# lucidrains/vit-pytorch

Hardware: AMD Instinct MI355X
Metric: images/sec (fwd+bwd) ViT-B/16 224^2 bf16 (higher is better)
Workload: dtype bf16

## Files before the change

include/vitk.h:

```cpp
#ifndef VITK_H
#define VITK_H

#include <stdint.h>
#include <stddef.h>

#ifdef __cplusplus
extern "C" {
#endif

#define VITK_VERSION 138

#define VITK_F32 0
#define VITK_BF16 1
#define VITK_F16 2

#define VITK_E_ARG (-1)
#define VITK_E_SHAPE (-2)
#define VITK_E_ALIGN (-3)
#define VITK_E_DTYPE (-4)
#define VITK_E_UNAVAILABLE (-5)
#define VITK_E_COMM (-6)

int vitk_version(void);
int vitk_half_type(void);
const char* vitk_last_error(void);

typedef struct vitk_rowmap { int64_t group, gstride, offset; } vitk_rowmap;

int vitk_layernorm_fwd(const void* x, int xdt, const void* w, const void* b, int wdt,
                       void* y, int ydt, float* mean, float* rstd,
                       int64_t rows, int64_t D, float eps,
                       vitk_rowmap imap, vitk_rowmap omap,
                       const void* add, int64_t add_group, int64_t add_off, void* stream);

int64_t vitk_layernorm_bwd_blocks(int64_t rows, int64_t D);
int vitk_layernorm_bwd(const void* dy, int dydt, const void* x, int xdt, const void* w, int wdt,
                       const float* mean, const float* rstd,
                       const float* gin, float* dx_f32, void* dx_t, int dxtdt,
                       float* partials, int colsum_dx,
                       int64_t rows, int64_t D,
                       vitk_rowmap dymap, vitk_rowmap xmap, vitk_rowmap dxmap, void* stream);
int vitk_layernorm_bwd_drop(const void* dy, int dydt, const void* x, int xdt, const void* w, int wdt,
                            const float* mean, const float* rstd, const float* gin, float* dx_f32, void* dx_t, int dxtdt,
                            float* partials, int colsum_dx, int64_t rows, int64_t D, vitk_rowmap dymap, vitk_rowmap xmap,
                            vitk_rowmap dxmap, float drop_p, uint32_t drop_seed, void* stream);
int vitk_layernorm_bwd_s16(const void* dy, int dydt, const void* x, int xdt, const void* w, int wdt, const float* mean,
                           const float* rstd, const void* gin, void* dx_t, int dxtdt, float* partials, int colsum_dx,
                           int64_t rows, int64_t D, vitk_rowmap dymap, vitk_rowmap xmap, vitk_rowmap dxmap, void* stream);

int vitk_layernorm_bwd_finalize(const float* partials, int64_t nblk, int64_t D, void* dw, void* db, int odt,
                                float* dcol, void* stream);
int vitk_layernorm_bwd_finalize_ex(const float* partials, int64_t nblk, int64_t D, void* dw, void* db, int odt,
                                   void* dcol, int dcol_dt, void* stream);

int vitk_colsum_partials(const float* partials, int64_t nparts, int64_t ld, int64_t cols,
                         void* out, int odt, int accumulate, void* stream);

int64_t vitk_colsum_ws_floats(int64_t rows, int64_t cols);
int vitk_colsum(const void* x, int xdt, int64_t rows, int64_t cols, int64_t ld,
                void* out, int odt, int accumulate, float* ws, void* stream);

#define VITK_EPI_NONE 0
#define VITK_EPI_BIAS 1
#define VITK_EPI_BIAS_GELU 2
#define VITK_EPI_RESID 3
#define VITK_EPI_RESID16 5
#define VITK_EPI_GELU_BWD 4
#define VITK_EPI_BIAS_GELU_DG 6
#define VITK_EPI_MUL_AUX 7
#define VITK_EPI_BIAS_GELU_DG8 8
#define VITK_EPI_MUL_AUX8 9

int vitk_gemm_nt_bf16(const void* A, int64_t lda, const void* W, int64_t ldw,
                      void* C, int64_t ldc, int64_t M, int64_t N, int64_t K,
                      int epilogue, const void* bias, const float* resid, void* aux, void* stream);

int64_t vitk_gemm_nt_colsum_rows(int64_t M, int64_t N, int64_t K, int64_t ldc);
int vitk_gemm_nt_bf16_mul_aux_colsum(const void* A, int64_t lda, const void* W, int64_t ldw, void* C, int64_t ldc,
                                     int64_t M, int64_t N, int64_t K, const void* aux, float* colsum_partials, void* stream);
int vitk_gemm_nt_bf16_mul_aux8_colsum(const void* A, int64_t lda, const void* W, int64_t ldw, void* C, int64_t ldc,
                                      int64_t M, int64_t N, int64_t K, const void* aux8, float* colsum_partials, void* stream);
int vitk_gemm_nt_plan(int64_t M, int64_t N, int64_t K, int64_t ldc, int32_t* out5);
int64_t vitk_pack_w_nt_bytes(int64_t rows, int64_t reduction);
int vitk_pack_w_nt(const void* W, int64_t ldw, int64_t N, int64_t K, void* out, void* out_t, void* stream);
int vitk_pack_w_nt_many(const void* const* W, const int64_t* ldw, const int64_t* N, const int64_t* K, void* const* out,
                        void* const* out_t, int64_t count, void* stream);
int vitk_gemm_nt_bf16_gelu_bwd_colsum(const void* A, int64_t lda, const void* W, int64_t ldw,
                                      void* C, int64_t ldc, int64_t M, int64_t N, int64_t K,
                                      void* aux, float* colsum_partials, void* stream);
int vitk_gemm_nt_bf16_drop(const void* A, int64_t lda, const void* W, int64_t ldw, void* C, int64_t ldc, int64_t M, int64_t N,
                           int64_t K, int epilogue, const void* bias, const float* resid, void* aux, float* colsum_partials,
                           float drop_p, uint32_t drop_seed, void* stream);

int vitk_gemm_nt_fp8(const void* A8, int64_t lda, const void* W8, int64_t ldw, void* C, int64_t ldc, int64_t M, int64_t N,
                     int64_t K, int epilogue, const void* bias, const float* resid, void* aux, float alpha, void* stream);
int vitk_fp8_amax_scale(const void* x, int dt, int64_t n, float* scale2, void* stream);
int vitk_quantize_fp8(const void* x, int dt, void* out, int64_t n, const float* scale_dev, float scale_host, void* stream);
int vitk_layernorm_fwd_fp8(const void* x, int xdt, const void* w, const void* b, int wdt, void* y, int ydt,
                           float* mean, float* rstd, int64_t rows, int64_t D, float eps, vitk_rowmap imap, vitk_rowmap omap,
                           const void* add, int64_t add_group, int64_t add_off, void* y8, const float* scale8,
                           uint32_t* amax64, void* stream);
int vitk_gemm_nt_fp8_ex(const void* A, int64_t lda, int a_is_fp8, const void* W, int64_t ldw, void* C, int64_t ldc, int64_t M,
                        int64_t N, int64_t K, int epilogue, const void* bias, const float* resid, void* aux, float alpha,
                        const float* alpha_a, const float* alpha_w, void* c8, const float* c8_scale, uint32_t* c8_amax64,
                        void* stream);
int vitk_fp8_update_scales(uint32_t* amax64, float* scales2, int64_t nslots, void* stream);
int vitk_gemm_nt_fp8_v2(const void* A, int64_t lda, int a_kind, const void* W, int64_t ldw, void* C, int64_t ldc, int64_t M,
                        int64_t N, int64_t K, int epilogue, const void* bias, const float* resid, void* aux,
                        float* colsum_partials, float alpha, const float* alpha_a, const float* alpha_w, void* c8,
                        const float* c8_scale, uint32_t* c8_amax64, int flags, void* stream);
int64_t vitk_gemm_nt_fp8_colsum_rows(int64_t M, int64_t N, int64_t K, int64_t ldc);
int vitk_quantize_fp8_delayed(const void* x, int dt, void* out8, int64_t n, const float* scale2, uint32_t* amax64, int fmt,
                              void* stream);
int vitk_fp8_update_scales_fmt(uint32_t* amax64, float* scales2, int64_t nslots, const float* fmax, void* stream);
int64_t vitk_gemm_tn_fp8_splits(int64_t M, int64_t N, int64_t K, int flags);
int vitk_gemm_tn_fp8(const void* dY8, int64_t ldy, const void* X8, int64_t ldx, void* dW, int odt, int64_t ldo, int accumulate,
                     int64_t M, int64_t N, int64_t K, float* ws, int64_t splits, const float* alpha_y, const float* alpha_x,
                     int flags, void* stream);

int64_t vitk_gemm_tn_splits(int64_t M, int64_t N, int64_t K);
int vitk_set_cu_reserve(int cus);
int vitk_get_cu_reserve(void);
int vitk_test_occupy_cus(int ncus, float ms, void* stream);
int vitk_gemm_tn_bf16(const void* dY, int64_t ldy, const void* X, int64_t ldx,
                      void* dW, int odt, int64_t ldo, int accumulate,
                      int64_t M, int64_t N, int64_t K, float* ws, int64_t splits, void* stream);
int64_t vitk_gemm_tn_pair_splits(int64_t M, int64_t N0, int64_t K0, int64_t N1, int64_t K1);
int vitk_gemm_tn_bf16_pair(const void* dY0, int64_t ldy0, const void* X0, int64_t ldx0, void* dW0, int64_t ldo0, int accumulate0,
                           int64_t N0, int64_t K0, const void* dY1, int64_t ldy1, const void* X1, int64_t ldx1, void* dW1,
                           int64_t ldo1, int accumulate1, int64_t N1, int64_t K1, int odt, int64_t M, float* ws, int64_t splits,
                           void* stream);

typedef struct vitk_mat { const void* p; int dt; int64_t s_b1, s_b2, s_row, s_col; } vitk_mat;
int vitk_gemm_generic(vitk_mat A, vitk_mat B, vitk_mat C, const void* bias, int bias_dt,
                      int64_t nb1, int64_t nb2, int64_t M, int64_t N, int64_t K,
                      float alpha, float beta, void* stream);

typedef struct vitk_bhnd { void* p; int64_t s_b, s_h, s_n; } vitk_bhnd;
int vitk_attn_fwd_bf16(vitk_bhnd q, vitk_bhnd k, vitk_bhnd v, vitk_bhnd o, float* lse,
                       int64_t B, int64_t H, int64_t N, int64_t d, float scale, void* stream);
int vitk_attn_bwd_bf16(vitk_bhnd q, vitk_bhnd k, vitk_bhnd v, vitk_bhnd o, vitk_bhnd dout,
                       const float* lse, float* delta,
                       vitk_bhnd dq, vitk_bhnd dk, vitk_bhnd dv,
                       int64_t B, int64_t H, int64_t N, int64_t d, float scale, void* stream);
int vitk_attn_fwd_bf16_drop(vitk_bhnd q, vitk_bhnd k, vitk_bhnd v, vitk_bhnd o, float* lse, int64_t B, int64_t H,
                            int64_t N, int64_t d, float scale, float drop_p, uint32_t drop_seed, void* stream);
int vitk_attn_bwd_bf16_drop(vitk_bhnd q, vitk_bhnd k, vitk_bhnd v, vitk_bhnd o, vitk_bhnd dout, const float* lse,
                            float* delta, vitk_bhnd dq, vitk_bhnd dk, vitk_bhnd dv, int64_t B, int64_t H, int64_t N,
                            int64_t d, float scale, float drop_p, uint32_t drop_seed, void* stream);
int vitk_split2(const float* x, void* hi, void* lo, int64_t n, void* stream);
int vitk_attn_fwd_x2(vitk_bhnd q_hi, vitk_bhnd q_lo, vitk_bhnd k_hi, vitk_bhnd k_lo, vitk_bhnd v_hi, vitk_bhnd v_lo, vitk_bhnd o_f32,
                     float* lse, int64_t B, int64_t H, int64_t N, int64_t d, float scale, void* stream);
int vitk_attn_bwd_x2(vitk_bhnd q_hi, vitk_bhnd q_lo, vitk_bhnd k_hi, vitk_bhnd k_lo, vitk_bhnd v_hi, vitk_bhnd v_lo, vitk_bhnd o_f32,
                     vitk_bhnd do_hi, vitk_bhnd do_lo, const float* lse, float* delta, vitk_bhnd dq_f32, vitk_bhnd dk_f32,
                     vitk_bhnd dv_f32, int64_t B, int64_t H, int64_t N, int64_t d, float scale, void* stream);
int vitk_dropout_keep(uint8_t* keep, int64_t rows, int64_t cols, float p, uint32_t seed, void* stream);

typedef struct vitk_hnd { void* p; int64_t s_h, s_n; } vitk_hnd;
int vitk_attn_varlen_fwd_bf16(vitk_hnd q, vitk_hnd k, vitk_hnd v, vitk_hnd o, float* lse,
                              const int32_t* cu_q, const int32_t* cu_k, const int32_t* blk_seg, const int32_t* blk_r0,
                              int64_t nblk, int64_t tq_total, int64_t H, int64_t d, float scale, void* stream);
int vitk_attn_varlen_bwd_bf16(vitk_hnd q, vitk_hnd k, vitk_hnd v, vitk_hnd o, vitk_hnd dout, const float* lse, float* delta,
                              vitk_hnd dq, vitk_hnd dk, vitk_hnd dv, const int32_t* cu_q, const int32_t* cu_k,
                              const int32_t* qblk_seg, const int32_t* qblk_r0, int64_t nqblk,
                              const int32_t* kblk_seg, const int32_t* kblk_r0, int64_t nkblk,
                              int64_t tq_total, int64_t H, int64_t d, float scale, void* stream);
int vitk_attn_varlen_fwd_bf16_drop(vitk_hnd q, vitk_hnd k, vitk_hnd v, vitk_hnd o, float* lse,
                                   const int32_t* cu_q, const int32_t* cu_k, const int32_t* blk_seg, const int32_t* blk_r0,
                                   int64_t nblk, int64_t tq_total, int64_t H, int64_t d, float scale, float drop_p,
                                   uint32_t drop_seed, void* stream);
int vitk_attn_varlen_bwd_bf16_drop(vitk_hnd q, vitk_hnd k, vitk_hnd v, vitk_hnd o, vitk_hnd dout, const float* lse, float* delta,
                                   vitk_hnd dq, vitk_hnd dk, vitk_hnd dv, const int32_t* cu_q, const int32_t* cu_k,
                                   const int32_t* qblk_seg, const int32_t* qblk_r0, int64_t nqblk,
                                   const int32_t* kblk_seg, const int32_t* kblk_r0, int64_t nkblk,
                                   int64_t tq_total, int64_t H, int64_t d, float scale, float drop_p, uint32_t drop_seed,
                                   void* stream);

int64_t vitk_rmsnorm_heads_rows(int64_t T, int64_t H);
int vitk_rmsnorm_heads_fwd(const void* x, int64_t ldx, const void* gamma, void* y, int64_t ldy, float* rnorm, int dt,
                           int64_t T, int64_t H, int64_t d, void* stream);
int vitk_rmsnorm_heads_bwd(const void* dy, int64_t lddy, const void* x, int64_t ldx, const void* gamma, const float* rnorm,
                           void* dx, int64_t lddx, void* dgamma, float* partials, int dt,
                           int64_t T, int64_t H, int64_t d, void* stream);

int vitk_softmax_fwd(const void* s, void* p, int dt, int64_t rows, int64_t cols, float scale, void* stream);
int vitk_softmax_bwd(const void* p, const void* dp, void* ds, int dt, int64_t rows, int64_t cols,
                     float scale, void* stream);

int vitk_patchify(const void* img, void* out, int dt, int64_t B, int64_t C, int64_t H, int64_t W,
                  int64_t p1, int64_t p2, void* stream);
int vitk_unpatchify(const void* dpatch, void* dimg, int dt, int64_t B, int64_t C, int64_t H, int64_t W,
                    int64_t p1, int64_t p2, void* stream);
int vitk_patch_ln_serves(int dt, int64_t C, int64_t H, int64_t W, int64_t p1, int64_t p2);
int64_t vitk_patch_ln_bwd_blocks(int64_t rows);
int vitk_patch_ln_fwd(const void* img, int dt, const void* w, const void* b, void* y, float* mean, float* rstd, int64_t B,
                      int64_t C, int64_t H, int64_t W, int64_t p1, int64_t p2, float eps, void* stream);
int vitk_patch_ln_bwd_params(const void* dy, const void* img, int dt, const float* mean, const float* rstd, float* partials,
                             int64_t B, int64_t C, int64_t H, int64_t W, int64_t p1, int64_t p2, void* stream);
int vitk_patchify_cpp(const void* img, void* out, int dt, int64_t C, int64_t H, int64_t W, int64_t p,
                      int64_t row0, int64_t ld, void* stream);
int vitk_unpatchify_cpp(const void* dpatch, void* dimg, int dt, int64_t C, int64_t H, int64_t W, int64_t p,
                        int64_t row0, int64_t ld, void* stream);
int vitk_gather_add2(const void* x, const void* A, const int32_t* ia, const void* B, const int32_t* ib, void* out, int dt,
                     int64_t T, int64_t D, void* stream);
int vitk_csr_rowsum(const void* g, int gdt, const int32_t* ptr, const int32_t* rows, void* out, int odt,
                    int64_t nseg, int64_t D, void* stream);
int vitk_gelu_fwd(const void* x, void* y, int dt, int64_t n, void* stream);
int vitk_gelu_bwd(const void* dy, const void* x, void* dx, int dt, int64_t n, void* stream);
int vitk_add_rows(const void* a, int adt, const void* b, int bdt, const void* bias, int biasdt,
                  void* out, int odt, int64_t rows, int64_t cols, void* stream);
int vitk_cast(const void* x, int xdt, void* y, int ydt, int64_t n, void* stream);
int vitk_cast_many(const void* const* src, void* const* dst, const int64_t* numel, int64_t count, int xdt, int ydt, void* stream);
int vitk_fold_many(const float* const* src, void* const* dst, const int64_t* nparts, const int64_t* ld, const int64_t* cols,
                   const int32_t* flags, int64_t count, void* stream);
int vitk_write_cls_rows(void* x, int xdt, const void* cls, const void* pos, int pdt,
                        int64_t B, int64_t N, int64_t D, int64_t ncls, void* stream);
int vitk_mean_pool_fwd(const void* x, int xdt, void* out, int odt, int64_t B, int64_t N, int64_t D, void* stream);
int vitk_mean_pool_bwd(const void* dout, int ddt, void* dx, int xdt, int64_t B, int64_t N, int64_t D, void* stream);
int vitk_dropout_fwd(const void* x, void* y, uint8_t* mask, int dt, int64_t n, float p,
                     uint64_t seed, uint64_t offset, void* stream);
int vitk_dropout_bwd(const void* dy, const uint8_t* mask, void* dx, int dt, int64_t n, float p, void* stream);
int vitk_copy_cols(const void* src, int64_t ld_src, void* dst, int64_t ld_dst, int dt, int64_t rows, int64_t cols_copy,
                   int64_t cols_dst, void* stream);
int vitk_split_bf16x3(const float* x, int64_t ldx, void* out, int64_t ld_out, int64_t block_stride, int64_t rows,
                      int64_t cols, int operand_b, void* stream);
int vitk_concat_tokens(const void* x, const void* front, const void* pos, void* out, int dt, int64_t B, int64_t Np,
                       int64_t F, int64_t D, void* stream);
int vitk_gather_tokens(const void* src, const int32_t* idx, void* dst, int dt, int64_t B, int64_t Np, int64_t Kp, int64_t D,
                       int scatter, void* stream);
int vitk_adam_step(void* param, const void* grad, int dt, float* exp_avg, float* exp_avg_sq, float* master, int64_t n,
                   float lr, float beta1, float beta2, float eps, float weight_decay, int decoupled, int64_t step,
                   float grad_scale, void* stream);
int vitk_transpose(const void* in, void* out, int dt, int64_t rows, int64_t cols, void* stream);

#define VITK_COMM_ID_BYTES 128
typedef void* vitk_comm_t;
int vitk_comm_unique_id(void* out128);
int vitk_comm_init(const void* id128, int rank, int world, vitk_comm_t* out);
int vitk_comm_allreduce(vitk_comm_t comm, void* buf, int64_t n, int dt, int average, void* stream);
int vitk_comm_destroy(vitk_comm_t comm);

#ifdef __cplusplus
}
#endif
#endif
```

vit_pytorch_amd/_lib.py:

```python
from __future__ import annotations

import ctypes as C
import os
import threading

HERE = os.path.dirname(os.path.abspath(__file__))
LIB_PATH = os.environ.get("VITK_LIB") or os.path.join(HERE, "libvitk.so")
LIB_PATH_F16 = (os.path.join(os.path.dirname(LIB_PATH), os.path.basename(LIB_PATH).replace("libvitk", "libvitk_f16", 1)) if os.environ.get("VITK_LIB")
                else os.path.join(HERE, "libvitk_f16.so"))

F32, BF16 = 0, 1
HALF_TYPE_F16 = 2
EPI_NONE, EPI_BIAS, EPI_BIAS_GELU, EPI_RESID, EPI_GELU_BWD, EPI_RESID16, EPI_BIAS_GELU_DG, EPI_MUL_AUX = 0, 1, 2, 3, 4, 5, 6, 7
EPI_BIAS_GELU_DG8, EPI_MUL_AUX8 = 8, 9
VITK_VERSION = 138


class RowMap(C.Structure):
    _fields_ = [("group", C.c_int64), ("gstride", C.c_int64), ("offset", C.c_int64)]


class Mat(C.Structure):
    _fields_ = [("p", C.c_void_p), ("dt", C.c_int), ("s_b1", C.c_int64), ("s_b2", C.c_int64),
                ("s_row", C.c_int64), ("s_col", C.c_int64)]


class HND(C.Structure):
    _fields_ = [("p", C.c_void_p), ("s_h", C.c_int64), ("s_n", C.c_int64)]


class BHND(C.Structure):
    _fields_ = [("p", C.c_void_p), ("s_b", C.c_int64), ("s_h", C.c_int64), ("s_n", C.c_int64)]


IDENT = RowMap(0, 0, 0)

_vp, _i, _i64, _f, _u64 = C.c_void_p, C.c_int, C.c_int64, C.c_float, C.c_uint64

SIGNATURES = {
    "vitk_version": (_i, []),
    "vitk_last_error": (C.c_char_p, []),
    "vitk_layernorm_fwd": (_i, [_vp, _i, _vp, _vp, _i, _vp, _i, _vp, _vp, _i64, _i64, _f, RowMap, RowMap, _vp, _i64, _i64, _vp]),
    "vitk_layernorm_bwd_blocks": (_i64, [_i64, _i64]),
    "vitk_layernorm_bwd": (_i, [_vp, _i, _vp, _i, _vp, _i, _vp, _vp, _vp, _vp, _vp, _i, _vp, _i, _i64, _i64, RowMap, RowMap, RowMap, _vp]),
    "vitk_layernorm_bwd_finalize": (_i, [_vp, _i64, _i64, _vp, _vp, _i, _vp, _vp]),
    "vitk_layernorm_bwd_finalize_ex": (_i, [_vp, _i64, _i64, _vp, _vp, _i, _vp, _i, _vp]),
    "vitk_colsum_partials": (_i, [_vp, _i64, _i64, _i64, _vp, _i, _i, _vp]),
    "vitk_colsum_ws_floats": (_i64, [_i64, _i64]),
    "vitk_colsum": (_i, [_vp, _i, _i64, _i64, _i64, _vp, _i, _i, _vp, _vp]),
    "vitk_gemm_nt_bf16": (_i, [_vp, _i64, _vp, _i64, _vp, _i64, _i64, _i64, _i64, _i, _vp, _vp, _vp, _vp]),
    "vitk_half_type": (_i, []),
    "vitk_adam_step": (_i, [_vp, _vp, _i, _vp, _vp, _vp, _i64, _f, _f, _f, _f, _f, _i, _i64, _f, _vp]),
    "vitk_gemm_nt_bf16_drop": (_i, [_vp, _i64, _vp, _i64, _vp, _i64, _i64, _i64, _i64, _i, _vp, _vp, _vp, _vp, _f, C.c_uint32, _vp]),
    "vitk_layernorm_bwd_drop": (_i, [_vp, _i, _vp, _i, _vp, _i, _vp, _vp, _vp, _vp, _vp, _i, _vp, _i, _i64, _i64, RowMap, RowMap, RowMap, _f, C.c_uint32, _vp]),
    "vitk_layernorm_bwd_s16": (_i, [_vp, _i, _vp, _i, _vp, _i, _vp, _vp, _vp, _vp, _i, _vp, _i, _i64, _i64, RowMap, RowMap, RowMap, _vp]),
    "vitk_gemm_nt_fp8": (_i, [_vp, _i64, _vp, _i64, _vp, _i64, _i64, _i64, _i64, _i, _vp, _vp, _vp, _f, _vp]),
    "vitk_fp8_amax_scale": (_i, [_vp, _i, _i64, _vp, _vp]),
    "vitk_quantize_fp8": (_i, [_vp, _i, _vp, _i64, _vp, _f, _vp]),
    "vitk_layernorm_fwd_fp8": (_i, [_vp, _i, _vp, _vp, _i, _vp, _i, _vp, _vp, _i64, _i64, _f, RowMap, RowMap, _vp, _i64, _i64, _vp, _vp, _vp, _vp]),
    "vitk_gemm_nt_fp8_ex": (_i, [_vp, _i64, _i, _vp, _i64, _vp, _i64, _i64, _i64, _i64, _i, _vp, _vp, _vp, _f, _vp, _vp, _vp, _vp, _vp, _vp]),
    "vitk_fp8_update_scales": (_i, [_vp, _vp, _i64, _vp]),
    "vitk_gemm_nt_fp8_v2": (_i, [_vp, _i64, _i, _vp, _i64, _vp, _i64, _i64, _i64, _i64, _i, _vp, _vp, _vp, _vp, _f, _vp, _vp, _vp, _vp, _vp, _i, _vp]),
    "vitk_gemm_nt_fp8_colsum_rows": (_i64, [_i64, _i64, _i64, _i64]),
    "vitk_quantize_fp8_delayed": (_i, [_vp, _i, _vp, _i64, _vp, _vp, _i, _vp]),
    "vitk_fp8_update_scales_fmt": (_i, [_vp, _vp, _i64, _vp, _vp]),
    "vitk_gemm_tn_fp8_splits": (_i64, [_i64, _i64, _i64, _i]),
    "vitk_gemm_tn_fp8": (_i, [_vp, _i64, _vp, _i64, _vp, _i, _i64, _i, _i64, _i64, _i64, _vp, _i64, _vp, _vp, _i, _vp]),
    "vitk_gemm_nt_colsum_rows": (_i64, [_i64, _i64, _i64, _i64]),
    "vitk_gemm_nt_plan": (_i, [_i64, _i64, _i64, _i64, _vp]),
    "vitk_comm_unique_id": (_i, [_vp]),
    "vitk_comm_init": (_i, [_vp, _i, _i, _vp]),
    "vitk_comm_allreduce": (_i, [_vp, _vp, _i64, _i, _i, _vp]),
    "vitk_comm_destroy": (_i, [_vp]),
    "vitk_pack_w_nt_bytes": (_i64, [_i64, _i64]),
    "vitk_pack_w_nt": (_i, [_vp, _i64, _i64, _i64, _vp, _vp, _vp]),
    "vitk_pack_w_nt_many": (_i, [_vp, _vp, _vp, _vp, _vp, _vp, _i64, _vp]),
    "vitk_gemm_nt_bf16_gelu_bwd_colsum": (_i, [_vp, _i64, _vp, _i64, _vp, _i64, _i64, _i64, _i64, _vp, _vp, _vp]),
    "vitk_gemm_nt_bf16_mul_aux_colsum": (_i, [_vp, _i64, _vp, _i64, _vp, _i64, _i64, _i64, _i64, _vp, _vp, _vp]),
    "vitk_gemm_nt_bf16_mul_aux8_colsum": (_i, [_vp, _i64, _vp, _i64, _vp, _i64, _i64, _i64, _i64, _vp, _vp, _vp]),
    "vitk_gemm_tn_splits": (_i64, [_i64, _i64, _i64]),
    "vitk_set_cu_reserve": (_i, [_i]),
    "vitk_get_cu_reserve": (_i, []),
    "vitk_test_occupy_cus": (_i, [_i, _f, _vp]),
    "vitk_gemm_tn_bf16": (_i, [_vp, _i64, _vp, _i64, _vp, _i, _i64, _i, _i64, _i64, _i64, _vp, _i64, _vp]),
    "vitk_gemm_tn_pair_splits": (_i64, [_i64, _i64, _i64, _i64, _i64]),
    "vitk_gemm_tn_bf16_pair": (_i, [_vp, _i64, _vp, _i64, _vp, _i64, _i, _i64, _i64, _vp, _i64, _vp, _i64, _vp, _i64, _i, _i64, _i64, _i, _i64, _vp, _i64, _vp]),
    "vitk_gemm_generic": (_i, [Mat, Mat, Mat, _vp, _i, _i64, _i64, _i64, _i64, _i64, _f, _f, _vp]),
    "vitk_attn_fwd_bf16": (_i, [BHND, BHND, BHND, BHND, _vp, _i64, _i64, _i64, _i64, _f, _vp]),
    "vitk_attn_bwd_bf16": (_i, [BHND, BHND, BHND, BHND, BHND, _vp, _vp, BHND, BHND, BHND, _i64, _i64, _i64, _i64, _f, _vp]),
    "vitk_attn_fwd_bf16_drop": (_i, [BHND, BHND, BHND, BHND, _vp, _i64, _i64, _i64, _i64, _f, _f, C.c_uint32, _vp]),
    "vitk_attn_bwd_bf16_drop": (_i, [BHND, BHND, BHND, BHND, BHND, _vp, _vp, BHND, BHND, BHND, _i64, _i64, _i64, _i64, _f, _f, C.c_uint32, _vp]),
    "vitk_split2": (_i, [_vp, _vp, _vp, _i64, _vp]),
    "vitk_attn_fwd_x2": (_i, [BHND] * 7 + [_vp, _i64, _i64, _i64, _i64, _f, _vp]),
    "vitk_attn_bwd_x2": (_i, [BHND] * 9 + [_vp, _vp, BHND, BHND, BHND, _i64, _i64, _i64, _i64, _f, _vp]),
    "vitk_dropout_keep": (_i, [_vp, _i64, _i64, _f, C.c_uint32, _vp]),
    "vitk_attn_varlen_fwd_bf16": (_i, [HND, HND, HND, HND, _vp, _vp, _vp, _vp, _vp, _i64, _i64, _i64, _i64, _f, _vp]),
    "vitk_attn_varlen_bwd_bf16": (_i, [HND, HND, HND, HND, HND, _vp, _vp, HND, HND, HND, _vp, _vp, _vp, _vp, _i64, _vp, _vp, _i64, _i64, _i64, _i64, _f, _vp]),
    "vitk_attn_varlen_fwd_bf16_drop": (_i, [HND, HND, HND, HND, _vp, _vp, _vp, _vp, _vp, _i64, _i64, _i64, _i64, _f, _f, C.c_uint32, _vp]),
    "vitk_attn_varlen_bwd_bf16_drop": (_i, [HND, HND, HND, HND, HND, _vp, _vp, HND, HND, HND, _vp, _vp, _vp, _vp, _i64, _vp, _vp, _i64, _i64, _i64, _i64, _f, _f, C.c_uint32, _vp]),
    "vitk_rmsnorm_heads_rows": (_i64, [_i64, _i64]),
    "vitk_rmsnorm_heads_fwd": (_i, [_vp, _i64, _vp, _vp, _i64, _vp, _i, _i64, _i64, _i64, _vp]),
    "vitk_rmsnorm_heads_bwd": (_i, [_vp, _i64, _vp, _i64, _vp, _vp, _vp, _i64, _vp, _vp, _i, _i64, _i64, _i64, _vp]),
    "vitk_softmax_fwd": (_i, [_vp, _vp, _i, _i64, _i64, _f, _vp]),
    "vitk_softmax_bwd": (_i, [_vp, _vp, _vp, _i, _i64, _i64, _f, _vp]),
    "vitk_patchify": (_i, [_vp, _vp, _i, _i64, _i64, _i64, _i64, _i64, _i64, _vp]),
    "vitk_unpatchify": (_i, [_vp, _vp, _i, _i64, _i64, _i64, _i64, _i64, _i64, _vp]),
    "vitk_patchify_cpp": (_i, [_vp, _vp, _i, _i64, _i64, _i64, _i64, _i64, _i64, _vp]),
    "vitk_unpatchify_cpp": (_i, [_vp, _vp, _i, _i64, _i64, _i64, _i64, _i64, _i64, _vp]),
    "vitk_patch_ln_serves": (_i, [_i, _i64, _i64, _i64, _i64, _i64]),
    "vitk_patch_ln_bwd_blocks": (_i64, [_i64]),
    "vitk_patch_ln_fwd": (_i, [_vp, _i, _vp, _vp, _vp, _vp, _vp, _i64, _i64, _i64, _i64, _i64, _i64, _f, _vp]),
    "vitk_patch_ln_bwd_params": (_i, [_vp, _vp, _i, _vp, _vp, _vp, _i64, _i64, _i64, _i64, _i64, _i64, _vp]),
    "vitk_gather_add2": (_i, [_vp, _vp, _vp, _vp, _vp, _vp, _i, _i64, _i64, _vp]),
    "vitk_csr_rowsum": (_i, [_vp, _i, _vp, _vp, _vp, _i, _i64, _i64, _vp]),
    "vitk_gelu_fwd": (_i, [_vp, _vp, _i, _i64, _vp]),
    "vitk_gelu_bwd": (_i, [_vp, _vp, _vp, _i, _i64, _vp]),
    "vitk_add_rows": (_i, [_vp, _i, _vp, _i, _vp, _i, _vp, _i, _i64, _i64, _vp]),
    "vitk_cast": (_i, [_vp, _i, _vp, _i, _i64, _vp]),
    "vitk_cast_many": (_i, [_vp, _vp, _vp, _i64, _i, _i, _vp]),
    "vitk_fold_many": (_i, [_vp, _vp, _vp, _vp, _vp, _vp, _i64, _vp]),
    "vitk_write_cls_rows": (_i, [_vp, _i, _vp, _vp, _i, _i64, _i64, _i64, _i64, _vp]),
    "vitk_mean_pool_fwd": (_i, [_vp, _i, _vp, _i, _i64, _i64, _i64, _vp]),
    "vitk_mean_pool_bwd": (_i, [_vp, _i, _vp, _i, _i64, _i64, _i64, _vp]),
    "vitk_dropout_fwd": (_i, [_vp, _vp, _vp, _i, _i64, _f, _u64, _u64, _vp]),
    "vitk_dropout_bwd": (_i, [_vp, _vp, _vp, _i, _i64, _f, _vp]),
    "vitk_copy_cols": (_i, [_vp, _i64, _vp, _i64, _i, _i64, _i64, _i64, _vp]),
    "vitk_split_bf16x3": (_i, [_vp, _i64, _vp, _i64, _i64, _i64, _i64, _i, _vp]),
    "vitk_concat_tokens": (_i, [_vp, _vp, _vp, _vp, _i, _i64, _i64, _i64, _i64, _vp]),
    "vitk_gather_tokens": (_i, [_vp, _vp, _vp, _i, _i64, _i64, _i64, _i64, _i, _vp]),
    "vitk_transpose": (_i, [_vp, _vp, _i, _i64, _i64, _vp]),
}

_lib = None
_lib_f16 = None


class VitkError(RuntimeError):
    pass


def _open(path: str, half_type: int):
    if not os.path.exists(path):
        raise VitkError(
            f"{path} not found: the HIP kernel library is not built. "
            "Build it with `python -c 'import __graft_entry__ as g; g.build()'` "
            "(or `python -m vit_pytorch_amd._build`). There is no CPU/eager fallback.")
    import torch
    lib = C.CDLL(path)
    for name, (res, args) in SIGNATURES.items():
        fn = getattr(lib, name)
        fn.restype = res
        fn.argtypes = args
    v = lib.vitk_version()
    if v != VITK_VERSION:
        raise VitkError(f"{os.path.basename(path)} version {v} != binding version {VITK_VERSION}; rebuild")
    if lib.vitk_half_type() != half_type:
        raise VitkError(f"{os.path.basename(path)} was built for the wrong 16-bit type; rebuild")
    return lib


def load():
    global _lib
    if _lib is None:
        _lib = _open(LIB_PATH, BF16)
    return _lib


def load_f16():
    global _lib_f16
    if _lib_f16 is None:
        _lib_f16 = _open(LIB_PATH_F16, HALF_TYPE_F16)
    return _lib_f16


_tls = threading.local()


def note_last_lib(lib):
    _tls.lib = lib


def check(rc: int, what: str = ""):
    if rc != 0:
        msg = (getattr(_tls, "lib", None) or load()).vitk_last_error().decode("utf-8", "replace")
        raise VitkError(f"{what}: vitk error {rc}: {msg}")
```

vit_pytorch_amd/csrc/gemm_bf16.hip:

```cpp
#include "common.h"
#include <atomic>
#include "gemm_nt_plan.h"
#include <stdlib.h>

namespace {

constexpr int BM = 128, BN = 128;
constexpr int NT_BK = 32;
constexpr int NT_TILE_BYTES = 128 * NT_BK * 2;
constexpr int NT_STAGE_BYTES = 2 * NT_TILE_BYTES;
constexpr int NXCD = 8;

__device__ __forceinline__ int xcd_swizzle(int b, int nwg) {
    const int q = nwg / NXCD, r = nwg % NXCD;
    const int xcd = b % NXCD, idx = b / NXCD;
    return (xcd < r ? xcd * (q + 1) : r * (q + 1) + (xcd - r) * q) + idx;
}

__device__ __forceinline__ void grouped_tile(int wg, int tiles_m, int tiles_n, int gn, int& tm, int& tn) {
    const int per_group = gn * tiles_m;
    const int g = wg / per_group;
    const int r = wg - g * per_group;
    const int rem = tiles_n - g * gn;
    const int w = rem < gn ? rem : gn;
    tm = r / w;
    tn = g * gn + (r - tm * w);
}

__device__ __forceinline__ int swz_f(int x) { return (0x1320 >> (4 * (x & 3))) & 3; }

template <int EPI>
__global__ __launch_bounds__(256) void gemm_nt_kernel(
    const __bf16* __restrict__ A, long long lda, const __bf16* __restrict__ W, long long ldw,
    void* __restrict__ Cv, long long ldc, int M, int N, int K,
    const __bf16* __restrict__ bias, const float* __restrict__ resid, __bf16* __restrict__ aux,
    int tiles_n, int nwg) {
    __shared__ __attribute__((aligned(16))) char lds[2 * NT_STAGE_BYTES];

    const int tid = threadIdx.x;
    const int lane = tid & 63;
    const int wave = tid >> 6;
    const int wm = wave >> 1, wn = wave & 1;
    const int wg = xcd_swizzle(blockIdx.x, nwg);
    const int tm = wg / tiles_n, tn = wg % tiles_n;
    const int m0 = tm * BM, n0 = tn * BN;

    const int srow = lane >> 2;
    const int spos = lane & 3;
    const int schunk = spos ^ swz_f(lane >> 4);
    const __bf16* a_src[2];
    const __bf16* w_src[2];
#pragma unroll
    for (int j = 0; j < 2; ++j) {
        const int rg = wave * 2 + j;
        int ar = m0 + rg * 16 + srow; ar = ar < M ? ar : M - 1;
        int wr = n0 + rg * 16 + srow; wr = wr < N ? wr : N - 1;
        a_src[j] = A + (long long)ar * lda + schunk * 8;
        w_src[j] = W + (long long)wr * ldw + schunk * 8;
    }
    auto stage = [&](int buf, int kt) {
        char* base = lds + buf * NT_STAGE_BYTES;
#pragma unroll
        for (int j = 0; j < 2; ++j) {
            const int rg = wave * 2 + j;
            __builtin_amdgcn_global_load_lds((const void __attribute__((address_space(1)))*)(a_src[j] + kt * NT_BK),
                                             (void __attribute__((address_space(3)))*)(base + rg * 1024), 16, 0, 0);
            __builtin_amdgcn_global_load_lds((const void __attribute__((address_space(1)))*)(w_src[j] + kt * NT_BK),
                                             (void __attribute__((address_space(3)))*)(base + NT_TILE_BYTES + rg * 1024), 16, 0, 0);
        }
    };

    const int fi = lane & 15, fg = lane >> 4;
    const int fpos = fg ^ swz_f(fi >> 2);
    const int a_off = (wm * 64 + fi) * 64 + fpos * 16;
    const int w_off = NT_TILE_BYTES + (wn * 64 + fi) * 64 + fpos * 16;

    f32x4 acc[4][4];
#pragma unroll
    for (int i = 0; i < 4; ++i)
#pragma unroll
        for (int j = 0; j < 4; ++j) acc[i][j] = f32x4{0.f, 0.f, 0.f, 0.f};

    const int nt = K / NT_BK;
    stage(0, 0);
    for (int t = 0; t < nt; ++t) {
        __syncthreads();
        if (t + 1 < nt) stage((t + 1) & 1, t + 1);
        const char* base = lds + (t & 1) * NT_STAGE_BYTES;
        bf16x8 xf[4], wf[4];
#pragma unroll
        for (int f = 0; f < 4; ++f) {
            xf[f] = *reinterpret_cast<const bf16x8*>(base + a_off + f * 1024);
            wf[f] = *reinterpret_cast<const bf16x8*>(base + w_off + f * 1024);
        }
#pragma unroll
        for (int fn = 0; fn < 4; ++fn)
#pragma unroll
            for (int fm = 0; fm < 4; ++fm)
                acc[fn][fm] = __builtin_amdgcn_mfma_f32_16x16x32_bf16(wf[fn], xf[fm], acc[fn][fm], 0, 0, 0);
    }

#pragma unroll
    for (int fm = 0; fm < 4; ++fm) {
        const int m = m0 + wm * 64 + fm * 16 + fi;
        if (m >= M) continue;
#pragma unroll
        for (int fn = 0; fn < 4; ++fn) {
            const int n = n0 + wn * 64 + fn * 16 + 4 * fg;
            if (n >= N) continue;
            f32x4 v = acc[fn][fm];
            const long long o = (long long)m * ldc + n;
            if constexpr (EPI == VITK_EPI_BIAS || EPI == VITK_EPI_BIAS_GELU) {
                v += load4<__bf16>(bias + n);
            }
            if constexpr (EPI == VITK_EPI_NONE || EPI == VITK_EPI_BIAS) {
                store4<__bf16>(reinterpret_cast<__bf16*>(Cv) + o, v);
            } else if constexpr (EPI == VITK_EPI_BIAS_GELU) {
                store4<__bf16>(aux + o, v);
                f32x4 gq;
#pragma unroll
                for (int e = 0; e < 4; ++e) gq[e] = gelu_erf(v[e]);
                store4<__bf16>(reinterpret_cast<__bf16*>(Cv) + o, gq);
            } else if constexpr (EPI == VITK_EPI_RESID) {
                if (bias) v += load4<__bf16>(bias + n);
                v += *reinterpret_cast<const f32x4*>(resid + o);
                *reinterpret_cast<f32x4*>(reinterpret_cast<float*>(Cv) + o) = v;
            } else if constexpr (EPI == VITK_EPI_GELU_BWD) {
                const f32x4 h = load4<__bf16>(aux + o);
#pragma unroll
                for (int e = 0; e < 4; ++e) v[e] *= gelu_erf_grad(h[e]);
                store4<__bf16>(reinterpret_cast<__bf16*>(Cv) + o, v);
            }
        }
    }
}

constexpr int TN_BKM = 32;
constexpr int TN_LD = 288;
constexpr int TN_TILE_BYTES = TN_BKM * TN_LD;
constexpr int TN_STAGE_BYTES = 2 * TN_TILE_BYTES;

__device__ __forceinline__ bf16x8 tr_frag(const char* tile, int off) {
    const s16x4 lo = __builtin_amdgcn_ds_read_tr16_b64_v4i16((s16x4 __attribute__((address_space(3)))*)(tile + off));
    const s16x4 hi = __builtin_amdgcn_ds_read_tr16_b64_v4i16((s16x4 __attribute__((address_space(3)))*)(tile + off + 16 * TN_LD));
    const s16x8 v = {lo[0], lo[1], lo[2], lo[3], hi[0], hi[1], hi[2], hi[3]};
    return __builtin_bit_cast(bf16x8, v);
}

__global__ __launch_bounds__(256) void gemm_tn_kernel(
    const __bf16* __restrict__ dY, long long ldy, const __bf16* __restrict__ X, long long ldx,
    float* __restrict__ ws, int M, int N, int K, int rows_per_split, int tiles_k, int nwg) {
    __shared__ __attribute__((aligned(16))) char lds[2 * TN_STAGE_BYTES];
    const int tid = threadIdx.x;
    const int lane = tid & 63;
    const int wave = tid >> 6;
    const int wn = wave >> 1, wk = wave & 1;
    const int lin = xcd_swizzle(blockIdx.x, (int)gridDim.x);
    const int split = lin / nwg;
    const int wg = lin % nwg;
    const int tn = wg / tiles_k, tk = wg % tiles_k;
    const int n0 = tn * BN, k0 = tk * BM;
    const int mbeg = split * rows_per_split;
    int mend = mbeg + rows_per_split; mend = mend < M ? mend : M;

    int srow[2], scol[2];
#pragma unroll
    for (int j = 0; j < 2; ++j) { const int c = tid + 256 * j; srow[j] = c >> 4; scol[j] = (c & 15) * 8; }
    const bf16x8 zero8 = {0, 0, 0, 0, 0, 0, 0, 0};
    bf16x8 ry[2], rx[2];
    auto gload = [&](int mb) {
#pragma unroll
        for (int j = 0; j < 2; ++j) {
            const int m = mb + srow[j];
            const bool mv = m < mend;
            ry[j] = (mv && n0 + scol[j] < N) ? *reinterpret_cast<const bf16x8*>(dY + (long long)m * ldy + n0 + scol[j]) : zero8;
            rx[j] = (mv && k0 + scol[j] < K) ? *reinterpret_cast<const bf16x8*>(X + (long long)m * ldx + k0 + scol[j]) : zero8;
        }
    };
    auto lstore = [&](int buf) {
        char* base = lds + buf * TN_STAGE_BYTES;
#pragma unroll
        for (int j = 0; j < 2; ++j) {
            *reinterpret_cast<bf16x8*>(base + srow[j] * TN_LD + scol[j] * 2) = ry[j];
            *reinterpret_cast<bf16x8*>(base + TN_TILE_BYTES + srow[j] * TN_LD + scol[j] * 2) = rx[j];
        }
    };

    const int fi = lane & 15, fg = lane >> 4;
    const int tr_off = (4 * fg + (fi >> 2)) * TN_LD + (fi & 3) * 8;
    const int y_off = tr_off + wn * 128;
    const int x_off = TN_TILE_BYTES + tr_off + wk * 128;

    f32x4 acc[4][4];
#pragma unroll
    for (int i = 0; i < 4; ++i)
#pragma unroll
        for (int j = 0; j < 4; ++j) acc[i][j] = f32x4{0.f, 0.f, 0.f, 0.f};

    const int nsteps = (mend - mbeg + TN_BKM - 1) / TN_BKM;
    if (nsteps > 0) {
        gload(mbeg);
        lstore(0);
        __syncthreads();
        for (int t = 0; t < nsteps; ++t) {
            if (t + 1 < nsteps) gload(mbeg + (t + 1) * TN_BKM);
            const char* base = lds + (t & 1) * TN_STAGE_BYTES;
            bf16x8 yf[4], xf[4];
#pragma unroll
            for (int f = 0; f < 4; ++f) {
                yf[f] = tr_frag(base, y_off + f * 32);
                xf[f] = tr_frag(base, x_off + f * 32);
            }
#pragma unroll
            for (int fn = 0; fn < 4; ++fn)
#pragma unroll
                for (int fk = 0; fk < 4; ++fk)
                    acc[fn][fk] = __builtin_amdgcn_mfma_f32_16x16x32_bf16(yf[fn], xf[fk], acc[fn][fk], 0, 0, 0);
            if (t + 1 < nsteps) lstore((t + 1) & 1);
            __syncthreads();
        }
    }
    float* out = ws + (long long)split * N * K;
#pragma unroll
    for (int fn = 0; fn < 4; ++fn)
#pragma unroll
        for (int r = 0; r < 4; ++r) {
            const int n = n0 + wn * 64 + fn * 16 + 4 * fg + r;
            if (n >= N) continue;
#pragma unroll
            for (int fk = 0; fk < 4; ++fk) {
                const int k = k0 + wk * 64 + fk * 16 + fi;
                if (k < K) out[(long long)n * K + k] = acc[fn][fk][r];
            }
        }
}

template <typename OT>
__global__ __launch_bounds__(256) void tn_reduce_kernel(const float* __restrict__ ws, int splits, long long NK, int K,
                                                         OT* __restrict__ out, long long ldo, int accumulate, long long slab_stride) {
    const long long i4 = ((long long)blockIdx.x * 256 + threadIdx.x) * 4;
    if (i4 >= NK) return;
    f32x4 s = *reinterpret_cast<const f32x4*>(ws + i4);
    for (int p = 1; p < splits; ++p) s += *reinterpret_cast<const f32x4*>(ws + (long long)p * slab_stride + i4);
    const long long n = i4 / K, k = i4 % K;
    OT* o = out + n * ldo + k;
    if (accumulate) s += load4<OT>(o);
    store4<OT>(o, s);
}


constexpr int L_BN = 256, L_BK = 64;

constexpr int P_BK = 32, P_STAGES = 4;
constexpr int P_TILE_BYTES = 256 * P_BK * 2;
constexpr int P_STAGE_BYTES = 2 * P_TILE_BYTES;
constexpr int P_LDS_BYTES = P_STAGES * P_STAGE_BYTES;

#define PP_BARRIER() do { __builtin_amdgcn_sched_barrier(0); __builtin_amdgcn_s_barrier(); __builtin_amdgcn_sched_barrier(0); } while (0)

template <int EPI, int FM, int EB = 2, int F8 = 0>
__global__ __launch_bounds__(512) void gemm_nt256pp_kernel(
    const void* __restrict__ Av, long long lda, const void* __restrict__ Wv, long long ldw,
    void* __restrict__ Cv, long long ldc, int M, int N, int K,
    const __bf16* __restrict__ bias, const float* __restrict__ resid, __bf16* __restrict__ aux,
    int tiles_n, int nwg, int group_n, float* __restrict__ csum, float alpha, unsigned drop_t, unsigned drop_seed, float inv_keep,
    const float* __restrict__ alpha_a, const float* __restrict__ alpha_w, F8Out f8) {
    const char* A = reinterpret_cast<const char*>(Av);
    const char* W = reinterpret_cast<const char*>(Wv);
    extern __shared__ __attribute__((aligned(16))) char lds[];
    const int tid = threadIdx.x;
    const int lane = tid & 63;
    const int wave = __builtin_amdgcn_readfirstlane(tid >> 6);
    const int wm = wave >> 2, wn = wave & 3;
    const bool grp_b = wave >= 4;
    const int wg = xcd_swizzle(blockIdx.x, nwg);
    int tm, tn;
    grouped_tile(wg, nwg / tiles_n, tiles_n, group_n, tm, tn);
    constexpr int WROWS = 16 * FM;
    const int m0 = tm * (2 * WROWS), n0 = tn * L_BN;

    const int srow = lane >> 2, spos = lane & 3;
    const int schunk = spos ^ swz_f(lane >> 4);
    const char* a_src[2];
    const char* w_src[2];
#pragma unroll
    for (int j = 0; j < 2; ++j) {
        int ar = m0 + (wave * 2 + j) * 16 + srow; ar = ar < M ? ar : M - 1;
        int wr = n0 + (wave * 2 + j) * 16 + srow; wr = wr < N ? wr : N - 1;
        a_src[j] = A + (long long)ar * lda * EB + schunk * 16;
        w_src[j] = W + (long long)wr * ldw * EB + schunk * 16;
    }
    auto stage_a = [&](int kt) {
        char* base = lds + (kt & 3) * P_STAGE_BYTES + wave * 2048;
#pragma unroll
        for (int j = 0; j < 2; ++j)
            __builtin_amdgcn_global_load_lds((const void __attribute__((address_space(1)))*)(a_src[j] + kt * 64),
                                             (void __attribute__((address_space(3)))*)(base + j * 1024), 16, 0, 0);
    };
    auto stage_w = [&](int kt) {
        char* base = lds + (kt & 3) * P_STAGE_BYTES + P_TILE_BYTES + wave * 2048;
#pragma unroll
        for (int j = 0; j < 2; ++j)
            __builtin_amdgcn_global_load_lds((const void __attribute__((address_space(1)))*)(w_src[j] + kt * 64),
                                             (void __attribute__((address_space(3)))*)(base + j * 1024), 16, 0, 0);
    };
    auto mma = [&](const bf16x8& wfr, const bf16x8& xfr, f32x4 c) -> f32x4 {
        if constexpr (EB == 2) {
            return __builtin_amdgcn_mfma_f32_16x16x32_bf16(wfr, xfr, c, 0, 0, 0);
        } else {
            typedef long l2 __attribute__((ext_vector_type(2)));
            const l2 w2 = __builtin_bit_cast(l2, wfr), x2 = __builtin_bit_cast(l2, xfr);
            if constexpr (F8 & 1) {
                c = __builtin_amdgcn_mfma_f32_16x16x32_fp8_bf8(w2[0], x2[0], c, 0, 0, 0);
                return __builtin_amdgcn_mfma_f32_16x16x32_fp8_bf8(w2[1], x2[1], c, 0, 0, 0);
            } else {
                c = __builtin_amdgcn_mfma_f32_16x16x32_fp8_fp8(w2[0], x2[0], c, 0, 0, 0);
                return __builtin_amdgcn_mfma_f32_16x16x32_fp8_fp8(w2[1], x2[1], c, 0, 0, 0);
            }
        }
    };
    auto mma128 = [&](const bf16x8& w0, const bf16x8& w1, const bf16x8& x0, const bf16x8& x1, f32x4 c) -> f32x4 {
        typedef int i4 __attribute__((ext_vector_type(4)));
        typedef int i8 __attribute__((ext_vector_type(8)));
        const i8 a = __builtin_shufflevector(__builtin_bit_cast(i4, w0), __builtin_bit_cast(i4, w1), 0, 1, 2, 3, 4, 5, 6, 7);
        const i8 b = __builtin_shufflevector(__builtin_bit_cast(i4, x0), __builtin_bit_cast(i4, x1), 0, 1, 2, 3, 4, 5, 6, 7);
        return __builtin_amdgcn_mfma_scale_f32_16x16x128_f8f6f4(a, b, c, 0 , (F8 & 1) ? 1 : 0 , 0, 0, 0, 0);
    };
    static_assert(F8 == 0 || EB == 1, "the e5m2 / K = 128 flavours are fp8 flavours");

    const int fi = lane & 15, fg = lane >> 4;
    const int fpos = fg ^ swz_f(fi >> 2);
    const int a_off = (wm * WROWS + fi) * 64 + fpos * 16;
    const int w_off = P_TILE_BYTES + (wn * 64 + fi) * 64 + fpos * 16;

    f32x4 acc[4][FM];
#pragma unroll
    for (int i = 0; i < 4; ++i)
#pragma unroll
        for (int j = 0; j < FM; ++j) acc[i][j] = f32x4{0.f, 0.f, 0.f, 0.f};

    const int nt = K * EB / 64;
    stage_a(0); stage_w(0);
    if (nt > 1) { stage_a(1); stage_w(1); }
    if (nt > 2) { stage_a(2); stage_w(2); }
    if (nt > 2) asm volatile("s_waitcnt vmcnt(8)" ::: "memory");
    else if (nt > 1) asm volatile("s_waitcnt vmcnt(4)" ::: "memory");
    else asm volatile("s_waitcnt vmcnt(0)" ::: "memory");
    PP_BARRIER();
    if (grp_b) PP_BARRIER();

    if constexpr ((F8 & 2) != 0) {
        bf16x8 hw[4], hx[FM];
        for (int j = 0; j < nt; ++j) {
            const char* base = lds + (j & 3) * P_STAGE_BYTES;
            const bool more = j + 3 < nt;
            const bool odd = (j & 1) != 0;
            bf16x8 wf[4], xf[4];
#pragma unroll
            for (int f = 0; f < 4; ++f) wf[f] = *reinterpret_cast<const bf16x8*>(base + w_off + f * 1024);
#pragma unroll
            for (int f = 0; f < 4; ++f) xf[f] = *reinterpret_cast<const bf16x8*>(base + a_off + f * 1024);
            if (more) stage_a(j + 3);
            asm volatile("s_waitcnt lgkmcnt(0)" ::: "memory");
            PP_BARRIER();
            if (odd) {
                __builtin_amdgcn_s_setprio(1);
#pragma unroll
                for (int fn = 0; fn < 4; ++fn)
#pragma unroll
                    for (int f = 0; f < 4; ++f)
                        acc[fn][f] = mma128(hw[fn], wf[fn], hx[f], xf[f], acc[fn][f]);
                __builtin_amdgcn_s_setprio(0);
            } else {
#pragma unroll
                for (int f = 0; f < 4; ++f) { hw[f] = wf[f]; hx[f] = xf[f]; }
            }
            PP_BARRIER();
#pragma unroll
            for (int f = 0; f < FM - 4; ++f) xf[f] = *reinterpret_cast<const bf16x8*>(base + a_off + (4 + f) * 1024);
            if (more) stage_w(j + 3);
            if (more) asm volatile("s_waitcnt vmcnt(8)" ::: "memory");
            else if (j + 2 < nt) asm volatile("s_waitcnt vmcnt(4)" ::: "memory");
            else asm volatile("s_waitcnt vmcnt(0)" ::: "memory");
            asm volatile("s_waitcnt lgkmcnt(0)" ::: "memory");
            PP_BARRIER();
            if (odd) {
                __builtin_amdgcn_s_setprio(1);
#pragma unroll
                for (int fn = 0; fn < 4; ++fn)
#pragma unroll
                    for (int f = 0; f < FM - 4; ++f)
                        acc[fn][4 + f] = mma128(hw[fn], wf[fn], hx[4 + f], xf[f], acc[fn][4 + f]);
                __builtin_amdgcn_s_setprio(0);
            } else {
#pragma unroll
                for (int f = 0; f < FM - 4; ++f) hx[4 + f] = xf[f];
            }
            PP_BARRIER();
        }
    } else
    for (int j = 0; j < nt; ++j) {
        const char* base = lds + (j & 3) * P_STAGE_BYTES;
        const bool more = j + 3 < nt;
        bf16x8 wf[4], xf[4];
#pragma unroll
        for (int f = 0; f < 4; ++f) wf[f] = *reinterpret_cast<const bf16x8*>(base + w_off + f * 1024);
#pragma unroll
        for (int f = 0; f < 4; ++f) xf[f] = *reinterpret_cast<const bf16x8*>(base + a_off + f * 1024);
        if (more) stage_a(j + 3);
        asm volatile("s_waitcnt lgkmcnt(0)" ::: "memory");
        PP_BARRIER();
        __builtin_amdgcn_s_setprio(1);
#pragma unroll
        for (int fn = 0; fn < 4; ++fn)
#pragma unroll
            for (int f = 0; f < 4; ++f)
                acc[fn][f] = mma(wf[fn], xf[f], acc[fn][f]);
        __builtin_amdgcn_s_setprio(0);
        PP_BARRIER();
#pragma unroll
        for (int f = 0; f < FM - 4; ++f) xf[f] = *reinterpret_cast<const bf16x8*>(base + a_off + (4 + f) * 1024);
        if (more) stage_w(j + 3);
        if (more) asm volatile("s_waitcnt vmcnt(8)" ::: "memory");
        else if (j + 2 < nt) asm volatile("s_waitcnt vmcnt(4)" ::: "memory");
        else asm volatile("s_waitcnt vmcnt(0)" ::: "memory");
        asm volatile("s_waitcnt lgkmcnt(0)" ::: "memory");
        PP_BARRIER();
        __builtin_amdgcn_s_setprio(1);
#pragma unroll
        for (int fn = 0; fn < 4; ++fn)
#pragma unroll
            for (int f = 0; f < FM - 4; ++f)
                acc[fn][4 + f] = mma(wf[fn], xf[f], acc[fn][4 + f]);
        __builtin_amdgcn_s_setprio(0);
        PP_BARRIER();
    }
    if (!grp_b) PP_BARRIER();
    if constexpr (EB == 1) {
        const float al = alpha * (alpha_a ? *alpha_a : 1.0f) * (alpha_w ? *alpha_w : 1.0f);
#pragma unroll
        for (int i = 0; i < 4; ++i)
#pragma unroll
            for (int jj = 0; jj < FM; ++jj) acc[i][jj] *= al;
    }

    __syncthreads();
    char* ep = lds + wave * 16384;
    const int mrow0 = m0 + wm * WROWS, ncol0 = n0 + wn * 64;
    if constexpr (EPI == VITK_EPI_RESID) {
        const int rr = lane >> 4, rc = lane & 15;
        const int ncol = ncol0 + rc * 4;
        f32x4 b4 = {0.f, 0.f, 0.f, 0.f};
        if (bias && ncol < N) b4 = load4<__bf16>(bias + ncol);
        constexpr int NF0 = 4, NF1 = FM - 4;
        f32x4 rpre[2][16];
        auto fetch_resid = [&](int hh) {
            const int nf = hh ? NF1 : NF0;
#pragma unroll
            for (int j = 0; j < 16; ++j) {
                const int m = mrow0 + hh * 64 + j * 4 + rr;
                rpre[hh][j] = f32x4{0.f, 0.f, 0.f, 0.f};
                if (j < nf * 4 && m < M && ncol < N) rpre[hh][j] = *reinterpret_cast<const f32x4*>(resid + (long long)m * ldc + ncol);
            }
        };
        fetch_resid(0);
#pragma unroll
        for (int hh = 0; hh < 2; ++hh) {
            const int nf = hh ? NF1 : NF0;
#pragma unroll
            for (int f4 = 0; f4 < 4; ++f4) {
                if (f4 < nf) {
                    const int row = f4 * 16 + fi;
#pragma unroll
                    for (int fn = 0; fn < 4; ++fn) {
                        const int c16 = fn * 4 + fg;
                        *reinterpret_cast<f32x4*>(ep + row * 256 + ((c16 ^ (row & 15)) * 16)) = acc[fn][hh * 4 + f4 < FM ? hh * 4 + f4 : 0];
                    }
                }
            }
            if (hh == 0) fetch_resid(1);
#pragma unroll
            for (int j = 0; j < 16; ++j) {
                if (j < nf * 4) {
                    const int row = j * 4 + rr;
                    f32x4 v = *reinterpret_cast<const f32x4*>(ep + row * 256 + ((rc ^ (row & 15)) * 16));
                    const int m = mrow0 + hh * 64 + row;
                    if (m < M && ncol < N) {
                        v += b4;
                        if (drop_t) {
                            const unsigned hrow = drop_row((unsigned)m, drop_seed);
#pragma unroll
                            for (int e = 0; e < 4; ++e) v[e] = drop_keep(hrow, (unsigned)(ncol + e), drop_t) ? v[e] * inv_keep : 0.f;
                        }
                        v += rpre[hh][j];
                        *reinterpret_cast<f32x4*>(reinterpret_cast<float*>(Cv) + (long long)m * ldc + ncol) = v;
                    }
                }
            }
        }
    } else {
        f32x4 b4[4];
#pragma unroll
        for (int fn = 0; fn < 4; ++fn) {
            b4[fn] = f32x4{0.f, 0.f, 0.f, 0.f};
            if constexpr (EPI == VITK_EPI_BIAS || EPI == VITK_EPI_BIAS_GELU) {
                const int n = ncol0 + fn * 16 + 4 * fg;
                if (n < N) b4[fn] = load4<__bf16>(bias + n);
            }
        }
        const int rr = lane >> 3, rc = lane & 7;
        const int ncol = ncol0 + rc * 8;
        bf16x8 hpre[2 * FM];
        if constexpr (EPI == VITK_EPI_GELU_BWD) {
#pragma unroll
            for (int j = 0; j < 2 * FM; ++j) {
                const int m = mrow0 + j * 8 + rr;
                hpre[j] = bf16x8{0, 0, 0, 0, 0, 0, 0, 0};
                if (m < M && ncol < N) hpre[j] = *reinterpret_cast<const bf16x8*>(aux + (long long)m * ldc + ncol);
            }
        }
#pragma unroll
        for (int fm = 0; fm < FM; ++fm) {
            const int row = fm * 16 + fi;
#pragma unroll
            for (int fn = 0; fn < 4; ++fn) {
                const int c16 = fn * 2 + (fg >> 1);
                const f32x4 v = acc[fn][fm] + b4[fn];
                const bf16x4 pk = {(__bf16)v[0], (__bf16)v[1], (__bf16)v[2], (__bf16)v[3]};
                *reinterpret_cast<bf16x4*>(ep + row * 128 + ((c16 ^ (row & 7)) * 16) + (((fg & 1) ^ ((row >> 3) & 1)) * 8)) = pk;
            }
        }
        float cs[8] = {0.f, 0.f, 0.f, 0.f, 0.f, 0.f, 0.f, 0.f};
        float f8max = 0.f;
#pragma unroll
        for (int j = 0; j < 2 * FM; ++j) {
            const int row = j * 8 + rr;
            bf16x8 v = *reinterpret_cast<const bf16x8*>(ep + row * 128 + ((rc ^ (row & 7)) * 16));
            if (j & 1) v = bf16x8{v[4], v[5], v[6], v[7], v[0], v[1], v[2], v[3]};
            const int m = mrow0 + row;
            if (m < M && ncol < N) {
                const long long o = (long long)m * ldc + ncol;
                if constexpr (EPI == VITK_EPI_NONE || EPI == VITK_EPI_BIAS) {
                    *reinterpret_cast<bf16x8*>(reinterpret_cast<__bf16*>(Cv) + o) = v;
                } else if constexpr (EPI == VITK_EPI_BIAS_GELU) {
                    *reinterpret_cast<bf16x8*>(aux + o) = v;
                    bf16x8 g8;
#pragma unroll
                    for (int e = 0; e < 8; e += 2) {
                        const f32x2 g2 = gelu_fast2(f32x2{(float)v[e], (float)v[e + 1]});
                        g8[e] = (__bf16)g2[0]; g8[e + 1] = (__bf16)g2[1];
                    }
                    if (drop_t) {
                        const unsigned hrow = drop_row((unsigned)m, drop_seed);
#pragma unroll
                        for (int e = 0; e < 8; ++e)
                            g8[e] = drop_keep(hrow, (unsigned)(ncol + e), drop_t) ? (__bf16)((float)g8[e] * inv_keep) : (__bf16)0.f;
                    }
                    if (Cv) *reinterpret_cast<bf16x8*>(reinterpret_cast<__bf16*>(Cv) + o) = g8;
                    if (f8.p || f8.amax) {
                        const f32x4 lo = {(float)g8[0], (float)g8[1], (float)g8[2], (float)g8[3]};
                        const f32x4 hi = {(float)g8[4], (float)g8[5], (float)g8[6], (float)g8[7]};
                        if (f8.p) {
                            const float sc8 = *f8.scale;
                            unsigned* d8 = reinterpret_cast<unsigned*>(f8.p + o);
                            d8[0] = pack_fp8x4(lo, sc8); d8[1] = pack_fp8x4(hi, sc8);
                        }
                        if (f8.amax) f8max = fmaxf(f8max, fmaxf(absmax4(lo), absmax4(hi)));
                    }
                } else if constexpr (EPI == VITK_EPI_GELU_BWD) {
                    const bf16x8 h8 = hpre[j];
                    bf16x8 g8;
                    float km[8];
                    if (drop_t) {
                        const unsigned hrow = drop_row((unsigned)m, drop_seed);
#pragma unroll
                        for (int e = 0; e < 8; ++e) km[e] = drop_keep(hrow, (unsigned)(ncol + e), drop_t) ? inv_keep : 0.f;
                    } else {
#pragma unroll
                        for (int e = 0; e < 8; ++e) km[e] = 1.f;
                    }
#pragma unroll
                    for (int e = 0; e < 8; e += 2) {
                        const f32x2 g2 = f32x2{(float)v[e], (float)v[e + 1]} * gelu_grad_fast2(f32x2{(float)h8[e], (float)h8[e + 1]}) * f32x2{km[e], km[e + 1]};
                        g8[e] = (__bf16)g2[0]; g8[e + 1] = (__bf16)g2[1];
                        cs[e] += (float)g8[e]; cs[e + 1] += (float)g8[e + 1];
                    }
                    *reinterpret_cast<bf16x8*>(reinterpret_cast<__bf16*>(Cv) + o) = g8;
                    if (f8.p || f8.amax) {
                        const f32x4 lo = {(float)g8[0], (float)g8[1], (float)g8[2], (float)g8[3]};
                        const f32x4 hi = {(float)g8[4], (float)g8[5], (float)g8[6], (float)g8[7]};
                        if (f8.p) {
                            const float sc8 = *f8.scale;
                            unsigned* d8 = reinterpret_cast<unsigned*>(f8.p + o);
                            d8[0] = pack_bf8x4(lo, sc8); d8[1] = pack_bf8x4(hi, sc8);
                        }
                        if (f8.amax) f8max = fmaxf(f8max, fmaxf(absmax4(lo), absmax4(hi)));
                    }
                }
            }
        }
        if constexpr (EPI == VITK_EPI_BIAS_GELU || EPI == VITK_EPI_GELU_BWD) {
            if (f8.amax) {
                f8max = wave_max(f8max);
                __syncthreads();
                float* red = reinterpret_cast<float*>(lds);
                if (lane == 0) red[wave] = f8max;
                __syncthreads();
                if (tid == 0) {
                    float m = red[0];
#pragma unroll
                    for (int k = 1; k < 8; ++k) m = fmaxf(m, red[k]);
                    atomicMax(f8.amax + (blockIdx.x & 63), __builtin_bit_cast(unsigned, m));
                }
            }
        }
        if constexpr (EPI == VITK_EPI_GELU_BWD) {
            if (csum) {
                float* cp = reinterpret_cast<float*>(ep);
#pragma unroll
                for (int e = 0; e < 8; ++e) cp[rr * 64 + rc * 8 + e] = cs[e];
                float t = 0.f;
#pragma unroll
                for (int r8 = 0; r8 < 8; ++r8) t += cp[r8 * 64 + lane];
                const int n = ncol0 + lane;
                if (n < N) csum[(long long)(tm * 2 + wm) * N + n] = t;
            }
        }
    }
}

template <typename Kern>
int set_max_lds(Kern kernel, int bytes) {
    return (int)hipFuncSetAttribute(reinterpret_cast<const void*>(kernel), hipFuncAttributeMaxDynamicSharedMemorySize, bytes);
}

}

namespace {
struct NtPlan { bool large; int fm; };
NtPlan nt_plan(int64_t M, int64_t N, int64_t K, int64_t ldc, const void* aux) {
    NtPlan pl;
    pl.large = (K % L_BK == 0) && M >= 1024 && N >= 256 && (N % 8 == 0) && (ldc % 8 == 0) && (!aux || aligned16(aux));
    pl.fm = 8;
    if (pl.large) {
        const long long tn_ = (N + L_BN - 1) / L_BN;
        const long long t8 = ((M + 255) / 256) * tn_, t7 = ((M + 223) / 224) * tn_;
        const long long cost8 = ((t8 + 255) / 256) * 8, cost7 = ((t7 + 255) / 256) * 7;
        if (cost7 * 10 <= cost8 * 9) pl.fm = 7;
    }
    return pl;
}
int gemm_nt_impl(const void* A, int64_t lda, const void* W, int64_t ldw, void* C, int64_t ldc, int64_t M, int64_t N, int64_t K,
                 int epilogue, const void* bias, const float* resid, void* aux, float* csum, void* stream, bool fp8 = false,
                 float alpha = 1.0f, float drop_p = 0.f, unsigned drop_seed = 0u, const float* alpha_a = nullptr,
                 const float* alpha_w = nullptr, F8Out f8 = F8Out{nullptr, nullptr, nullptr}, int f8kind = 0);
}

extern "C" int vitk_gemm_nt_bf16(const void* A, int64_t lda, const void* W, int64_t ldw, void* C, int64_t ldc, int64_t M,
                                 int64_t N, int64_t K, int epilogue, const void* bias, const float* resid, void* aux,
                                 void* stream) {
    return gemm_nt_impl(A, lda, W, ldw, C, ldc, M, N, K, epilogue, bias, resid, aux, nullptr, stream);
}

extern "C" int vitk_gemm_nt_bf16_drop(const void* A, int64_t lda, const void* W, int64_t ldw, void* C, int64_t ldc, int64_t M, int64_t N,
                                      int64_t K, int epilogue, const void* bias, const float* resid, void* aux, float* colsum_partials,
                                      float drop_p, uint32_t drop_seed, void* stream) {
    if (colsum_partials && (epilogue != VITK_EPI_GELU_BWD || vitk_gemm_nt_colsum_rows(M, N, K, ldc) == 0))
        VITK_FAIL(VITK_E_SHAPE, "gemm_nt_bf16_drop: column sums come with the GELU_BWD epilogue of the 256-row kernel only");
    return gemm_nt_impl(A, lda, W, ldw, C, ldc, M, N, K, epilogue, bias, resid, aux, colsum_partials, stream, false, 1.0f, drop_p, drop_seed);
}

extern "C" int vitk_gemm_nt_fp8_ex(const void* A, int64_t lda, int a_is_fp8, const void* W, int64_t ldw, void* C, int64_t ldc, int64_t M,
                                   int64_t N, int64_t K, int epilogue, const void* bias, const float* resid, void* aux, float alpha,
                                   const float* alpha_a, const float* alpha_w, void* c8, const float* c8_scale, uint32_t* c8_amax64,
                                   void* stream) {
    const F8Out f8{(unsigned char*)c8, c8_scale, (unsigned*)c8_amax64};
    return gemm_nt_impl(A, lda, W, ldw, C, ldc, M, N, K, epilogue, bias, resid, aux, nullptr, stream, a_is_fp8 != 0, alpha, 0.f, 0u,
                        alpha_a, alpha_w, f8);
}

extern "C" int vitk_gemm_nt_fp8(const void* A, int64_t lda, const void* W, int64_t ldw, void* C, int64_t ldc, int64_t M, int64_t N,
                               int64_t K, int epilogue, const void* bias, const float* resid, void* aux, float alpha, void* stream) {
    return gemm_nt_impl(A, lda, W, ldw, C, ldc, M, N, K, epilogue, bias, resid, aux, nullptr, stream, true, alpha);
}

extern "C" int vitk_gemm_nt_fp8_v2(const void* A, int64_t lda, int a_kind, const void* W, int64_t ldw, void* C, int64_t ldc, int64_t M,
                                   int64_t N, int64_t K, int epilogue, const void* bias, const float* resid, void* aux,
                                   float* colsum_partials, float alpha, const float* alpha_a, const float* alpha_w, void* c8,
                                   const float* c8_scale, uint32_t* c8_amax64, int flags, void* stream) {
    if (a_kind < 0 || a_kind > 2) VITK_FAIL(VITK_E_ARG, "gemm_nt_fp8_v2: a_kind is 0 (16-bit), 1 (e4m3) or 2 (e5m2), got %d", a_kind);
    if (flags & ~1) VITK_FAIL(VITK_E_ARG, "gemm_nt_fp8_v2: unknown flags 0x%x", (unsigned)flags);
    if (a_kind == 0 && (flags & 1)) VITK_FAIL(VITK_E_ARG, "gemm_nt_fp8_v2: the K = 128 instruction takes 1-byte operands");
    if ((flags & 1) && (K % 128)) VITK_FAIL(VITK_E_SHAPE, "gemm_nt_fp8_v2: the K = 128 flavour needs K %% 128 == 0 (K = %lld)", (long long)K);
    if (colsum_partials && (epilogue != VITK_EPI_GELU_BWD || vitk_gemm_nt_fp8_colsum_rows(M, N, K, ldc) == 0))
        VITK_FAIL(VITK_E_SHAPE, "gemm_nt_fp8_v2: column sums come with the GELU_BWD epilogue of the 256-row kernel only");
    const F8Out f8{(unsigned char*)c8, c8_scale, (unsigned*)c8_amax64};
    return gemm_nt_impl(A, lda, W, ldw, C, ldc, M, N, K, epilogue, bias, resid, aux, colsum_partials, stream, a_kind != 0, alpha, 0.f, 0u,
                        alpha_a, alpha_w, f8, (a_kind == 2 ? 1 : 0) | ((flags & 1) ? 2 : 0));
}

extern "C" int64_t vitk_gemm_nt_fp8_colsum_rows(int64_t M, int64_t N, int64_t K, int64_t ldc) {
    if (M <= 0 || N <= 0 || K <= 0 || (K % 64)) return 0;
    const NtPlan pl = nt_plan(M, N, K, ldc, nullptr);
    if (!pl.large) return 0;
    return 2 * ((M + 32 * pl.fm - 1) / (32 * pl.fm));
}

static int64_t nt_persist_colsum_rows(const NtpPlan& q, int64_t M, int64_t N, int64_t K, int64_t ldc);
extern "C" int64_t vitk_gemm_nt_colsum_rows(int64_t M, int64_t N, int64_t K, int64_t ldc) {
    if (M <= 0 || N <= 0 || K <= 0) return 0;
    const NtpPlan q = ntp_plan(M, N, K, ldc, nullptr);
    if (q.ok) return nt_persist_colsum_rows(q, M, N, K, ldc);
    const NtPlan pl = nt_plan(M, N, K, ldc, nullptr);
    if (!pl.large) return 0;
    return 2 * ((M + 32 * pl.fm - 1) / (32 * pl.fm));
}

extern "C" int vitk_gemm_nt_plan(int64_t M, int64_t N, int64_t K, int64_t ldc, int32_t* out5) {
    if (!out5) VITK_FAIL(VITK_E_ARG, "gemm_nt_plan: null output");
    for (int i = 0; i < 5; ++i) out5[i] = 0;
    if (M <= 0 || N <= 0 || K <= 0) return 0;
    const NtpPlan q = ntp_plan(M, N, K, ldc, nullptr);
    if (q.ok) { out5[0] = 1; out5[1] = q.tm_main; out5[2] = q.tail_tm; out5[3] = q.grid; out5[4] = q.tiles_n; }
    return 0;
}

extern "C" int vitk_gemm_nt_bf16_gelu_bwd_colsum(const void* A, int64_t lda, const void* W, int64_t ldw, void* C, int64_t ldc,
                                                 int64_t M, int64_t N, int64_t K, void* aux, float* colsum_partials, void* stream) {
    if (!colsum_partials) VITK_FAIL(VITK_E_ARG, "gemm_nt_bf16_gelu_bwd_colsum: null partials");
    if (vitk_gemm_nt_colsum_rows(M, N, K, ldc) == 0 || (aux && !aligned16(aux)))
        VITK_FAIL(VITK_E_SHAPE, "gemm_nt_bf16_gelu_bwd_colsum: shape not served by the 256-row kernel (vitk_gemm_nt_colsum_rows() == 0)");
    return gemm_nt_impl(A, lda, W, ldw, C, ldc, M, N, K, VITK_EPI_GELU_BWD, nullptr, nullptr, aux, colsum_partials, stream);
}

extern "C" int vitk_gemm_nt_bf16_mul_aux_colsum(const void* A, int64_t lda, const void* W, int64_t ldw, void* C, int64_t ldc, int64_t M,
                                                int64_t N, int64_t K, const void* aux, float* colsum_partials, void* stream) {
    if (!aux) VITK_FAIL(VITK_E_ARG, "gemm_nt_bf16_mul_aux_colsum: null pointer");
    if (colsum_partials && vitk_gemm_nt_colsum_rows(M, N, K, ldc) == 0)
        VITK_FAIL(VITK_E_SHAPE, "gemm_nt_bf16_mul_aux_colsum: shape not served by the persistent kernel (vitk_gemm_nt_colsum_rows() == 0)");
    return gemm_nt_impl(A, lda, W, ldw, C, ldc, M, N, K, VITK_EPI_MUL_AUX, nullptr, nullptr, const_cast<void*>(aux), colsum_partials, stream);
}

extern "C" int vitk_gemm_nt_bf16_mul_aux8_colsum(const void* A, int64_t lda, const void* W, int64_t ldw, void* C, int64_t ldc, int64_t M,
                                                 int64_t N, int64_t K, const void* aux8, float* colsum_partials, void* stream) {
    if (!aux8) VITK_FAIL(VITK_E_ARG, "gemm_nt_bf16_mul_aux8_colsum: null pointer");
    if (colsum_partials && vitk_gemm_nt_colsum_rows(M, N, K, ldc) == 0)
        VITK_FAIL(VITK_E_SHAPE, "gemm_nt_bf16_mul_aux8_colsum: shape not served by the persistent kernel (vitk_gemm_nt_colsum_rows() == 0)");
    return gemm_nt_impl(A, lda, W, ldw, C, ldc, M, N, K, VITK_EPI_MUL_AUX8, nullptr, nullptr, const_cast<void*>(aux8), colsum_partials, stream);
}

constexpr unsigned NTW_EPIS = 0xffu;
static int ntw_tiles_m(const NtpPlan& q, int64_t M, int64_t N, int64_t K, int epilogue, int grid = 0) {
    if (epilogue == VITK_EPI_BIAS_GELU_DG8) epilogue = VITK_EPI_BIAS_GELU_DG;
    if (epilogue == VITK_EPI_MUL_AUX8) epilogue = VITK_EPI_MUL_AUX;
    const char* e = vitk_switch("VITK_NT_W128");
    const unsigned mask = e ? (unsigned)strtoul(e, nullptr, 0) : NTW_EPIS;
    if (!q.ok || !((mask >> epilogue) & 1u) || !gemm_ntw_serves(M, N, K)) return 0;
    return gemm_ntw_split(M, N, K, grid > 0 ? grid : q.grid);
}
static int64_t nt_persist_colsum_rows(const NtpPlan& q, int64_t M, int64_t N, int64_t K, int64_t ldc) {
    const int tmw = ntw_tiles_m(q, M, N, K, VITK_EPI_MUL_AUX);
    if (tmw == 0) return ntp_colsum_rows(q);
    const int64_t rest = M - 256LL * tmw;
    return 2LL * tmw + (rest > 0 ? ntp_colsum_rows(ntp_plan(rest, N, K, ldc, nullptr)) : 0);
}
static int nt_persist_dispatch(const NtpPlan& q, const void* A, int64_t lda, const void* W, int64_t ldw, void* C, int64_t ldc, int64_t M, int64_t N,
                               int64_t K, int epilogue, const void* bias, const float* resid, void* aux, float* csum, unsigned drop_t,
                               unsigned drop_seed, float inv_keep, void* stream) {
    const int reserve = vitk_get_cu_reserve();
    int grid_w = q.grid - (reserve + 7) / 8 * 8;
    if (grid_w < q.grid / 4) grid_w = q.grid / 4 / 8 * 8;
    const int tmw = ntw_tiles_m(q, M, N, K, epilogue == VITK_EPI_GELU_BWD ? VITK_EPI_MUL_AUX : epilogue, csum ? 0 : grid_w);
    const int64_t asz = (epilogue == VITK_EPI_BIAS_GELU_DG8 || epilogue == VITK_EPI_MUL_AUX8) ? 1 : 2;
    if (tmw == 0 || (drop_t && !(epilogue == VITK_EPI_GELU_BWD && csum)))
        return gemm_ntp_launch(q, A, lda, W, ldw, C, ldc, M, N, K, epilogue, bias, resid, aux, csum, drop_t, drop_seed, inv_keep, stream);
    const int64_t rows_w = 256LL * tmw, rest = M - rows_w;
    int rc;
    if (drop_t) {
        NtpPlan q1 = q;
        q1.tm_main = tmw; q1.tail_tm = 0; q1.n_main = tmw * q1.tiles_n; q1.n_tail = 0;
        rc = gemm_ntp_launch(q1, A, lda, W, ldw, C, ldc, rows_w, N, K, epilogue, bias, resid, aux, csum, drop_t, drop_seed, inv_keep, stream);
    } else {
        if (256LL * (lda > ldw ? lda : ldw) * 2 + K * 2 >= (1LL << 31)) VITK_FAIL(VITK_E_SHAPE, "gemm_nt_bf16: row stride too large (lda %lld, ldw %lld)", (long long)lda, (long long)ldw);
        rc = gemm_ntw_launch(tmw, grid_w, A, lda, W, ldw, C, ldc, N, K, epilogue, bias, resid, aux, csum, 0, 0, stream);
    }
    if (rc != 0 || rest <= 0) return rc;
    const NtpPlan q2 = ntp_plan(rest, N, K, ldc, aux);
    if (!q2.ok) VITK_FAIL(VITK_E_SHAPE, "gemm_nt_bf16: internal: the row split left %lld rows the persistent kernel does not take", (long long)rest);
    const int64_t csz = epilogue == VITK_EPI_RESID ? 4 : 2;
    return gemm_ntp_launch(q2, (const char*)A + rows_w * lda * 2, lda, W, ldw, (char*)C + rows_w * ldc * csz, ldc, rest, N, K, epilogue, bias,
                           resid ? (const float*)((const char*)resid + rows_w * ldc * csz) : nullptr, aux ? (char*)aux + rows_w * ldc * asz : nullptr,
                           csum ? csum + 2LL * tmw * N : nullptr, drop_t, drop_seed, inv_keep, stream, (unsigned)rows_w);
}

namespace {
int gemm_nt_impl(const void* A, int64_t lda, const void* W, int64_t ldw, void* C, int64_t ldc, int64_t M, int64_t N, int64_t K,
                 int epilogue, const void* bias, const float* resid, void* aux, float* csum, void* stream, bool fp8, float alpha,
                 float drop_p, unsigned drop_seed, const float* alpha_a, const float* alpha_w, F8Out f8, int f8kind) {
    if (f8kind && !fp8) VITK_FAIL(VITK_E_ARG, "gemm_nt: e5m2 / K = 128 flavours need 1-byte operands");
    if ((f8kind & 1) && epilogue != VITK_EPI_NONE && epilogue != VITK_EPI_GELU_BWD)
        VITK_FAIL(VITK_E_ARG, "gemm_nt_fp8: e5m2 operands (gradients) come with the NONE and GELU_BWD epilogues only (got %d)", epilogue);
    if ((f8.p || f8.amax) && epilogue != VITK_EPI_BIAS_GELU && epilogue != VITK_EPI_GELU_BWD)
        VITK_FAIL(VITK_E_ARG, "gemm_nt: the fp8 side output exists in the BIAS_GELU (e4m3) and GELU_BWD (e5m2) epilogues only");
    if (f8.p && (!f8.scale || (ldc & 7))) VITK_FAIL(VITK_E_ARG, "gemm_nt: fp8 side output needs a scale and ldc %% 8 == 0");
    const bool c_optional = fp8 && epilogue == VITK_EPI_BIAS_GELU && f8.p;
    if (!A || !W || (!C && !c_optional)) VITK_FAIL(VITK_E_ARG, "gemm_nt_bf16: null pointer");
    if (!(drop_p >= 0.f && drop_p < 1.f)) VITK_FAIL(VITK_E_ARG, "gemm_nt_bf16: dropout p must be in [0, 1) (got %g)", (double)drop_p);
    const unsigned drop_t = drop_thresh(drop_p);
    const float inv_keep = 1.0f / (1.0f - drop_p);
    if (fp8 && ((lda & 15) || (ldw & 15) || (K % 64)))
        VITK_FAIL(VITK_E_ALIGN, "gemm_nt_fp8: K %% 64 == 0 and lda, ldw %% 16 == 0 required");
    if (M <= 0 || N <= 0 || K <= 0 || (K % NT_BK) || (N & 3) || M > (1 << 30) || N > (1 << 30))
        VITK_FAIL(VITK_E_SHAPE, "gemm_nt_bf16: need K %% 32 == 0 and N %% 4 == 0 (M=%lld N=%lld K=%lld)", (long long)M, (long long)N, (long long)K);
    if ((lda & 7) || (ldw & 7) || (ldc & 3) || !aligned16(A) || !aligned16(W) || !aligned16(C) || (bias && !aligned8(bias)) ||
        (resid && !aligned16(resid)) || (aux && !aligned8(aux)))
        VITK_FAIL(VITK_E_ALIGN, "gemm_nt_bf16: lda/ldw %% 8, ldc %% 4 and 16-byte aligned pointers required");
    if (ldw == 0 && (fp8 || f8.p || f8.amax)) VITK_FAIL(VITK_E_ARG, "gemm_nt: a K-blocked W (ldw == 0) goes with 16-bit operands only");
    if (!fp8 && !f8.p && !f8.amax) {
        const NtpPlan q = ntp_plan(M, N, K, ldc, aux);
        const unsigned epis = vitk_exp("VITK_NTP_EPIS") ? (unsigned)atoi(vitk_exp("VITK_NTP_EPIS")) : 0x1fu;
        const bool dg_out = epilogue == VITK_EPI_BIAS_GELU_DG || epilogue == VITK_EPI_BIAS_GELU_DG8;
        if (dg_out || epilogue == VITK_EPI_MUL_AUX || epilogue == VITK_EPI_MUL_AUX8) {
            if (!q.ok) VITK_FAIL(VITK_E_SHAPE, "gemm_nt_bf16: EPI_BIAS_GELU_DG(8) / EPI_MUL_AUX(8) are served by the persistent kernel only (vitk_gemm_nt_plan() says which shapes)");
            if (!aux || drop_t || (dg_out && !bias)) VITK_FAIL(VITK_E_ARG, "gemm_nt_bf16: EPI_BIAS_GELU_DG(8) needs bias and aux, EPI_MUL_AUX(8) aux; no fused dropout");
            return nt_persist_dispatch(q, A, lda, W, ldw, C, ldc, M, N, K, epilogue, bias, resid, aux, csum, 0u, 0u, 1.0f, stream);
        }
        if (epilogue == VITK_EPI_RESID16) {
            if (!q.ok) VITK_FAIL(VITK_E_SHAPE, "gemm_nt_bf16: EPI_RESID16 is served by the persistent kernel only (vitk_gemm_nt_plan() says which shapes)");
            if (!resid || !aligned8(resid) || drop_t) VITK_FAIL(VITK_E_ARG, "gemm_nt_bf16: EPI_RESID16 needs an 8-byte aligned 16-bit resid and no dropout");
            return nt_persist_dispatch(q, A, lda, W, ldw, C, ldc, M, N, K, epilogue, bias, resid, aux, csum, 0u, 0u, 1.0f, stream);
        }
        if (q.ok && epilogue >= 0 && epilogue <= 4 && (((epis >> epilogue) & 1u) || epilogue == VITK_EPI_GELU_BWD)) {
            switch (epilogue) {
                case VITK_EPI_NONE: break;
                case VITK_EPI_BIAS: if (!bias) VITK_FAIL(VITK_E_ARG, "gemm_nt_bf16: EPI_BIAS needs bias"); break;
                case VITK_EPI_BIAS_GELU: if (!bias || !aux) VITK_FAIL(VITK_E_ARG, "gemm_nt_bf16: EPI_BIAS_GELU needs bias and aux"); break;
                case VITK_EPI_RESID: if (!resid) VITK_FAIL(VITK_E_ARG, "gemm_nt_bf16: EPI_RESID needs resid"); break;
                case VITK_EPI_GELU_BWD: if (!aux) VITK_FAIL(VITK_E_ARG, "gemm_nt_bf16: EPI_GELU_BWD needs aux"); break;
                default: VITK_FAIL(VITK_E_ARG, "gemm_nt_bf16: bad epilogue %d", epilogue);
            }
            if (drop_t && epilogue != VITK_EPI_RESID && epilogue != VITK_EPI_BIAS_GELU && epilogue != VITK_EPI_GELU_BWD)
                VITK_FAIL(VITK_E_SHAPE, "gemm_nt_bf16: fused dropout exists for the RESID / BIAS_GELU / GELU_BWD epilogues only");
            return nt_persist_dispatch(q, A, lda, W, ldw, C, ldc, M, N, K, epilogue, bias, resid, aux, csum, drop_t, drop_seed, inv_keep, stream);
        }
    }
    if (ldw == 0) VITK_FAIL(VITK_E_SHAPE, "gemm_nt_bf16: a K-blocked W (ldw == 0, vitk_pack_w_nt) is read by the persistent kernel only (vitk_gemm_nt_plan() says which shapes it serves)");
    const NtPlan pl = nt_plan(M, N, K, ldc, aux);
    const bool large = pl.large;
    const int fm = pl.fm;
    if (fp8 && !large) VITK_FAIL(VITK_E_SHAPE, "gemm_nt_fp8: served by the 256-row kernel only (M >= 1024, N >= 256, N %% 8 == 0)");
    if ((f8.p || f8.amax) && !large) VITK_FAIL(VITK_E_SHAPE, "gemm_nt: the fp8 side output is served by the 256-row kernel only");
    if (drop_t && (!large || (epilogue != VITK_EPI_RESID && epilogue != VITK_EPI_BIAS_GELU && epilogue != VITK_EPI_GELU_BWD)))
        VITK_FAIL(VITK_E_SHAPE, "gemm_nt_bf16: fused dropout exists in the 256-row kernel for the RESID / BIAS_GELU / GELU_BWD epilogues only");
    const int tbm = large ? 32 * fm : BM, tbn = large ? L_BN : BN;
    const int tiles_m = (int)((M + tbm - 1) / tbm), tiles_n = (int)((N + tbn - 1) / tbn);
    const long long nwg = (long long)tiles_m * tiles_n;
    if (nwg > 0x7fffffffLL) VITK_FAIL(VITK_E_SHAPE, "gemm_nt_bf16: grid too large");
    hipStream_t st = (hipStream_t)stream;
    int group_n = tiles_n;
    if (large && tiles_n > 8) group_n = (tiles_n + (tiles_n + 5) / 6 - 1) / ((tiles_n + 5) / 6);
    if (vitk_exp("VITK_GROUP_N")) group_n = atoi(vitk_exp("VITK_GROUP_N")) > 0 ? atoi(vitk_exp("VITK_GROUP_N")) : tiles_n;
    if (group_n > tiles_n) group_n = tiles_n;
#define NT_LAUNCH_F8(E, F, FK) do { \
            static const int rc8__ = set_max_lds(gemm_nt256pp_kernel<E, F, 1, FK>, P_LDS_BYTES); \
            if (rc8__ != 0) VITK_FAIL(rc8__, "gemm_nt_fp8: cannot enable %d B of LDS", P_LDS_BYTES); \
            hipLaunchKernelGGL((gemm_nt256pp_kernel<E, F, 1, FK>), dim3((unsigned)nwg), dim3(512), P_LDS_BYTES, st, A, (long long)lda, \
                W, (long long)ldw, C, (long long)ldc, (int)M, (int)N, (int)K, (const __bf16*)bias, resid, (__bf16*)aux, tiles_n, (int)nwg, group_n, csum, alpha, drop_t, drop_seed, inv_keep, alpha_a, alpha_w, f8); \
        } while (0)
#define NT_LAUNCH_PP(E, F) do { \
        if (fp8) { \
            if constexpr (E == VITK_EPI_NONE || E == VITK_EPI_GELU_BWD) { \
                if (f8kind == 1) NT_LAUNCH_F8(E, F, 1); else if (f8kind == 3) NT_LAUNCH_F8(E, F, 3); \
                else if (f8kind == 2) NT_LAUNCH_F8(E, F, 2); else NT_LAUNCH_F8(E, F, 0); \
            } else { \
                if (f8kind == 2) NT_LAUNCH_F8(E, F, 2); else NT_LAUNCH_F8(E, F, 0); \
            } \
        } else { \
            static const int rc__ = set_max_lds(gemm_nt256pp_kernel<E, F, 2>, P_LDS_BYTES); \
            if (rc__ != 0) VITK_FAIL(rc__, "gemm_nt_bf16: cannot enable %d B of LDS", P_LDS_BYTES); \
            hipLaunchKernelGGL((gemm_nt256pp_kernel<E, F, 2>), dim3((unsigned)nwg), dim3(512), P_LDS_BYTES, st, A, (long long)lda, \
                W, (long long)ldw, C, (long long)ldc, (int)M, (int)N, (int)K, (const __bf16*)bias, resid, (__bf16*)aux, tiles_n, (int)nwg, group_n, csum, 1.0f, drop_t, drop_seed, inv_keep, nullptr, nullptr, f8); \
        } \
    } while (0)
#define NT_LAUNCH(E) do { \
    if (large && fm == 7) NT_LAUNCH_PP(E, 7); \
    else if (large) NT_LAUNCH_PP(E, 8); \
    else { \
        hipLaunchKernelGGL((gemm_nt_kernel<E>), dim3((unsigned)nwg), dim3(256), 0, st, (const __bf16*)A, (long long)lda, \
            (const __bf16*)W, (long long)ldw, C, (long long)ldc, (int)M, (int)N, (int)K, (const __bf16*)bias, resid, (__bf16*)aux, tiles_n, (int)nwg); \
    } } while (0)
    switch (epilogue) {
        case VITK_EPI_NONE: NT_LAUNCH(VITK_EPI_NONE); break;
        case VITK_EPI_BIAS:
            if (!bias) VITK_FAIL(VITK_E_ARG, "gemm_nt_bf16: EPI_BIAS needs bias");
            NT_LAUNCH(VITK_EPI_BIAS); break;
        case VITK_EPI_BIAS_GELU:
            if (!bias || !aux) VITK_FAIL(VITK_E_ARG, "gemm_nt_bf16: EPI_BIAS_GELU needs bias and aux");
            NT_LAUNCH(VITK_EPI_BIAS_GELU); break;
        case VITK_EPI_RESID:
            if (!resid) VITK_FAIL(VITK_E_ARG, "gemm_nt_bf16: EPI_RESID needs resid");
            NT_LAUNCH(VITK_EPI_RESID); break;
        case VITK_EPI_GELU_BWD:
            if (!aux) VITK_FAIL(VITK_E_ARG, "gemm_nt_bf16: EPI_GELU_BWD needs aux");
            NT_LAUNCH(VITK_EPI_GELU_BWD); break;
        default: VITK_FAIL(VITK_E_ARG, "gemm_nt_bf16: bad epilogue %d", epilogue);
    }
#undef NT_LAUNCH
#undef NT_LAUNCH_PP
#undef NT_LAUNCH_F8
    VITK_CHECK_LAUNCH("gemm_nt_bf16");
    return 0;
}
}


bool gemm_tn_w128_serves(int64_t M, int64_t N, int64_t K, int64_t ldy, int64_t ldx, int64_t splits);
int gemm_tn_w128_launch2(const void* dY0, int64_t ldy0, const void* X0, int64_t ldx0, int64_t N0, int64_t K0, const void* dY1, int64_t ldy1,
                         const void* X1, int64_t ldx1, int64_t N1, int64_t K1, float* ws, int64_t M, int64_t splits, void* stream);
int gemm_tn_w128_launch(const void* dY, int64_t ldy, const void* X, int64_t ldx, float* ws, int64_t M, int64_t N, int64_t K,
                        int64_t splits, void* stream);

static bool tn_large(int64_t M, int64_t N, int64_t K) { return M >= 4096 && N >= 256 && K >= 256; }

static std::atomic<int> g_cu_reserve{0};
extern "C" int vitk_set_cu_reserve(int cus) {
    if (cus < 0 || cus > 192) VITK_FAIL(VITK_E_ARG, "set_cu_reserve: 0 .. 192 (got %d)", cus);
    g_cu_reserve.store(cus);
    return 0;
}
extern "C" int vitk_get_cu_reserve(void) { return g_cu_reserve.load(); }

int64_t tn_pick_splits(int64_t tiles, int64_t M, int cus, long long slab_elems, double us_per_row, int64_t min_rows) {
    const int64_t max_by_rows = (M + min_rows - 1) / min_rows;
    int64_t best = 1;
    double best_c = 1e30;
    for (int64_t s = 1; s <= 64 && s <= max_by_rows; ++s) {
        const int64_t rounds = (tiles * s + cus - 1) / cus;
        const double job = (double)M / (double)s * us_per_row + 8.0;
        const double fold = (double)s * (double)slab_elems * 8.0 / 5.0e6;
        const double c = (double)rounds * job + fold;
        if (c < best_c - 1e-9) { best_c = c; best = s; }
    }
    return best;
}

extern "C" int64_t vitk_gemm_tn_splits(int64_t M, int64_t N, int64_t K) {
    if (tn_large(M, N, K)) {
        const int64_t tiles = ((N + 255) / 256) * ((K + 255) / 256);
        return tn_pick_splits(tiles, M, 256 - g_cu_reserve.load(), (long long)N * K, 0.024, 512);
    }
    const int64_t tiles = ((N + BN - 1) / BN) * ((K + BM - 1) / BM);
    int64_t s = (768 + tiles - 1) / tiles;
    const int64_t max_by_rows = (M + 255) / 256;
    if (s > max_by_rows) s = max_by_rows;
    if (s > 64) s = 64;
    if (s < 1) s = 1;
    return s;
}

extern "C" int vitk_gemm_tn_bf16(const void* dY, int64_t ldy, const void* X, int64_t ldx, void* dW, int odt, int64_t ldo,
                                 int accumulate, int64_t M, int64_t N, int64_t K, float* ws, int64_t splits, void* stream) {
    if (!dY || !X || !dW || !ws) VITK_FAIL(VITK_E_ARG, "gemm_tn_bf16: null pointer");
    if (M <= 0 || N <= 0 || K <= 0 || (N & 7) || (K & 7) || splits < 1 || splits > 65535 || M > (1 << 30))
        VITK_FAIL(VITK_E_SHAPE, "gemm_tn_bf16: need N %% 8 == 0, K %% 8 == 0 (M=%lld N=%lld K=%lld)", (long long)M, (long long)N, (long long)K);
    if ((ldy & 7) || (ldx & 7) || (ldo & 3) || !aligned16(dY) || !aligned16(X) || !aligned16(dW) || !aligned16(ws))
        VITK_FAIL(VITK_E_ALIGN, "gemm_tn_bf16: ldy/ldx %% 8, ldo %% 4 and 16-byte aligned pointers required");
    hipStream_t st = (hipStream_t)stream;
    if (tn_large(M, N, K) && gemm_tn_w128_serves(M, N, K, ldy, ldx, splits)) {
        const int rc = gemm_tn_w128_launch(dY, ldy, X, ldx, ws, M, N, K, splits, stream);
        if (rc != 0) return rc;
    } else {
        const int tiles_n = (int)((N + BN - 1) / BN), tiles_k = (int)((K + BM - 1) / BM);
        const int nwg = tiles_n * tiles_k;
        long long rps = (M + splits - 1) / splits;
        rps = (rps + TN_BKM - 1) / TN_BKM * TN_BKM;
        hipLaunchKernelGGL(gemm_tn_kernel, dim3((unsigned)(nwg * splits)), dim3(256), 0, st, (const __bf16*)dY, (long long)ldy,
                           (const __bf16*)X, (long long)ldx, ws, (int)M, (int)N, (int)K, (int)rps, tiles_k, nwg);
    }
    VITK_CHECK_LAUNCH("gemm_tn_bf16");
    const long long NK = (long long)N * K;
    const unsigned blocks = (unsigned)((NK / 4 + 255) / 256);
    VITK_DISPATCH_DT(odt, OT, hipLaunchKernelGGL((tn_reduce_kernel<OT>), dim3(blocks), dim3(256), 0, st, ws, (int)splits, NK, (int)K,
                                                  (OT*)dW, (long long)ldo, accumulate, NK));
    VITK_CHECK_LAUNCH("gemm_tn_reduce");
    return 0;
}

extern "C" int64_t vitk_gemm_tn_pair_splits(int64_t M, int64_t N0, int64_t K0, int64_t N1, int64_t K1) {
    if (!tn_large(M, N0, K0) || !tn_large(M, N1, K1) || (N0 & 7) || (K0 & 7) || (N1 & 7) || (K1 & 7)) return 0;
    if (vitk_switch("VITK_TN_PAIR") && atoi(vitk_switch("VITK_TN_PAIR")) == 0) return 0;
    const int64_t tiles = ((N0 + 255) / 256) * ((K0 + 255) / 256) + ((N1 + 255) / 256) * ((K1 + 255) / 256);
    const int64_t s = tn_pick_splits(tiles, M, 256 - g_cu_reserve.load(), (long long)N0 * K0 + (long long)N1 * K1, 0.024, 512);
    const int64_t ldmax = (N0 > K0 ? N0 : K0) > (N1 > K1 ? N1 : K1) ? (N0 > K0 ? N0 : K0) : (N1 > K1 ? N1 : K1);
    if (!gemm_tn_w128_serves(M, N0, K0, ldmax, ldmax, s)) return 0;
    return s;
}

extern "C" int vitk_gemm_tn_bf16_pair(const void* dY0, int64_t ldy0, const void* X0, int64_t ldx0, void* dW0, int64_t ldo0, int accumulate0,
                                      int64_t N0, int64_t K0, const void* dY1, int64_t ldy1, const void* X1, int64_t ldx1, void* dW1,
                                      int64_t ldo1, int accumulate1, int64_t N1, int64_t K1, int odt, int64_t M, float* ws, int64_t splits,
                                      void* stream) {
    if (!dY0 || !X0 || !dW0 || !dY1 || !X1 || !dW1 || !ws) VITK_FAIL(VITK_E_ARG, "gemm_tn_bf16_pair: null pointer");
    if (splits < 1 || splits != vitk_gemm_tn_pair_splits(M, N0, K0, N1, K1))
        VITK_FAIL(VITK_E_SHAPE, "gemm_tn_bf16_pair: splits must be vitk_gemm_tn_pair_splits(M, N0, K0, N1, K1) (0 = pair not served)");
    if ((ldy0 & 7) || (ldx0 & 7) || (ldo0 & 3) || (ldy1 & 7) || (ldx1 & 7) || (ldo1 & 3) || !aligned16(dY0) || !aligned16(X0) || !aligned16(dW0) ||
        !aligned16(dY1) || !aligned16(X1) || !aligned16(dW1) || !aligned16(ws))
        VITK_FAIL(VITK_E_ALIGN, "gemm_tn_bf16_pair: ldy/ldx %% 8, ldo %% 4 and 16-byte aligned pointers required");
    if (!gemm_tn_w128_serves(M, N0, K0, ldy0 > ldy1 ? ldy0 : ldy1, ldx0 > ldx1 ? ldx0 : ldx1, splits))
        VITK_FAIL(VITK_E_SHAPE, "gemm_tn_bf16_pair: row strides beyond the kernel's 32-bit offsets");
    const int rc = gemm_tn_w128_launch2(dY0, ldy0, X0, ldx0, N0, K0, dY1, ldy1, X1, ldx1, N1, K1, ws, M, splits, stream);
    if (rc != 0) return rc;
    hipStream_t st = (hipStream_t)stream;
    const long long NK0 = (long long)N0 * K0, NK1 = (long long)N1 * K1, stride = NK0 + NK1;
    VITK_DISPATCH_DT(odt, OT, hipLaunchKernelGGL((tn_reduce_kernel<OT>), dim3((unsigned)((NK0 / 4 + 255) / 256)), dim3(256), 0, st, ws, (int)splits, NK0,
                                                  (int)K0, (OT*)dW0, (long long)ldo0, accumulate0, stride));
    VITK_DISPATCH_DT(odt, OT, hipLaunchKernelGGL((tn_reduce_kernel<OT>), dim3((unsigned)((NK1 / 4 + 255) / 256)), dim3(256), 0, st, ws + NK0, (int)splits, NK1,
                                                  (int)K1, (OT*)dW1, (long long)ldo1, accumulate1, stride));
    VITK_CHECK_LAUNCH("gemm_tn_pair_reduce");
    return 0;
}
```

vit_pytorch_amd/csrc/gemm_nt_plan.h:

```cpp
#pragma once
#include <stdint.h>

struct NtpPlan {
    bool ok;
    int tiles_n;
    int group_n;
    int tm_main;
    int tail_tm;
    int n_main, n_tail;
    int nt;
    int grid;
};

NtpPlan ntp_plan(int64_t M, int64_t N, int64_t K, int64_t ldc, const void* aux);
static inline int64_t ntp_colsum_rows(const NtpPlan& pl) { return 2 * ((int64_t)pl.tm_main + pl.tail_tm); }

int gemm_ntp_launch(const NtpPlan& pl, const void* A, int64_t lda, const void* W, int64_t ldw, void* C, int64_t ldc, int64_t M,
                    int64_t N, int64_t K, int epilogue, const void* bias, const float* resid, void* aux, float* csum, unsigned drop_t, unsigned drop_seed,
                    float inv_keep, void* stream, unsigned drop_m0 = 0);

bool gemm_ntw_serves(int64_t M, int64_t N, int64_t K);
int gemm_ntw_split(int64_t M, int64_t N, int64_t K, int grid);
int gemm_ntw_launch(int tiles_m, int grid, const void* A, int64_t lda, const void* W, int64_t ldw, void* C, int64_t ldc,
                    int64_t N, int64_t K, int epilogue, const void* bias, const void* resid, void* aux, float* csum, int abl, int dbg, void* stream);
```

vit_pytorch_amd/csrc/gemm_nt_w128.hip:

```cpp
#include "common.h"
#include "gemm_nt_plan.h"
#include "gemm_nt_epi.h"
#include <stdlib.h>
#include <type_traits>

#ifdef VITK_HALF_IS_F16
#define NTW_MFMA_ASM "v_mfma_f32_16x16x32_f16"
#else
#define NTW_MFMA_ASM "v_mfma_f32_16x16x32_bf16"
#endif

namespace {

constexpr int V_TILE = 256 * 64;
constexpr int V_STAGE = 2 * V_TILE;
constexpr int V_RING = 4 * V_STAGE;
constexpr int V_LDS_MAX = V_RING + 32768;
constexpr int X_ASLOT = 256 * 128;
constexpr int X_WBASE = 3 * X_ASLOT;
constexpr int X_LDS = X_WBASE + 4 * V_TILE;

#define V_PIN() __builtin_amdgcn_sched_barrier(0)

__device__ __forceinline__ int v_swz(int x) { return (0x1320 >> (4 * (x & 3))) & 3; }

__device__ __forceinline__ void v_grouped_tile(int t, int tiles_m, int tiles_n, int gn, int& tm, int& tn) {
    const int per_group = gn * tiles_m;
    const int g = t / per_group;
    const int r = t - g * per_group;
    const int rem = tiles_n - g * gn;
    const int w = rem < gn ? rem : gn;
    tm = r / w;
    tn = g * gn + (r - tm * w);
}

struct NtwArgs {
    const char* A; long long lda;
    const char* W; long long ldw;
    void* C; long long ldc;
    int M, N, K;
    const __bf16* bias; const void* resid; __bf16* aux; float* csum;
    int tiles_n, group_n, tiles_m, n_tiles, nt;
    int dbg;
};

template <int OFF> __device__ __forceinline__ bf16x8 v_rd(unsigned lds_addr) {
    bf16x8 v;
    asm volatile("ds_read_b128 %0, %1 offset:%2" : "=v"(v) : "v"(lds_addr), "n"(OFF) : "memory");
    return v;
}
#ifdef NTW_PROBE
typedef float v_f32x16 __attribute__((ext_vector_type(16)));
#ifdef VITK_HALF_IS_F16
#define NTW_MFMA32_ASM "v_mfma_f32_32x32x16_f16"
#else
#define NTW_MFMA32_ASM "v_mfma_f32_32x32x16_bf16"
#endif
__device__ __forceinline__ void v_mfma32(v_f32x16& c, const bf16x8& a, const bf16x8& b) {
    asm volatile("" NTW_MFMA32_ASM " %0, %1, %2, %0" : "+a"(c) : "v"(a), "v"(b));
}
#endif
template <bool Z> __device__ __forceinline__ void v_mfma(f32x4& c, const bf16x8& a, const bf16x8& b) {
    if constexpr (Z) asm volatile("" NTW_MFMA_ASM " %0, %1, %2, 0" : "=a"(c) : "v"(a), "v"(b));
    else asm volatile("" NTW_MFMA_ASM " %0, %1, %2, %0" : "+a"(c) : "v"(a), "v"(b));
}

__device__ __forceinline__ void v_gload_bf16x4(bf16x4& d, const __bf16* p) { asm volatile("global_load_dwordx2 %0, %1, off" : "=v"(d) : "v"(p) : "memory"); }

template <int EPI, int ABL, int AW>
__global__ __launch_bounds__(256) void gemm_ntw_kernel(const NtwArgs p) {
    extern __shared__ __attribute__((aligned(16))) char lds[];
    constexpr bool F32OUT = (EPI == VITK_EPI_RESID);
    const int tid = threadIdx.x;
    const int lane = tid & 63;
    const int wave = __builtin_amdgcn_readfirstlane(tid >> 6);
    const int wm = wave >> 1, wn = wave & 1;

    const int xcd = blockIdx.x & 7, l0 = blockIdx.x >> 3, L = gridDim.x >> 3;
    const int ms = (int)(((long long)xcd * p.n_tiles) >> 3), count = (int)(((long long)(xcd + 1) * p.n_tiles) >> 3) - ms;
    if (l0 >= count) return;
    if ((p.dbg >> 8) && (l0 & 1)) { for (int i = (p.dbg >> 8) & 0xff; i > 0; --i) __builtin_amdgcn_s_sleep(127); }
    auto decode = [&](int idx, int& m0, int& n0, int& mt) {
        int tn;
        v_grouped_tile(ms + idx, p.tiles_m, p.tiles_n, p.group_n, mt, tn);
        m0 = mt * 256; n0 = tn * 256;
    };

    const int srow = lane >> 2, spos = lane & 3;
    const int schunk = spos ^ v_swz(lane >> 4);
    int avo[4], wvo[4];
#pragma unroll
    for (int j = 0; j < 4; ++j) {
        if constexpr (AW) avo[j] = (int)(((long long)(64 * wave + (lane >> 3)) * p.lda + (((lane & 7) ^ (4 * (j & 1) + (lane >> 4))) * 8)) * 2);
        else avo[j] = (int)(((long long)(64 * wave + 16 * j + srow) * p.lda + schunk * 8) * 2);
        wvo[j] = p.ldw == 0 ? (4 * wave + j) * 1024 + lane * 16 : (int)(((long long)(64 * wave + 4 * srow + j) * p.ldw + schunk * 8) * 2);
    }
    const int a_rows8 = (int)(p.lda * 16);
    const int w_kstride = p.ldw == 0 ? V_TILE : 64;
    __amdgpu_buffer_rsrc_t a_rs, w_rs;
    int a_so = 0, w_so = 0;
    auto setup_a = [&](int idx) __attribute__((always_inline)) {
        if (idx < count) {
            int m0, n0, mt;
            decode(idx, m0, n0, mt);
            const long long abytes = (255LL * p.lda + p.K) * 2;
            a_rs = __builtin_amdgcn_make_buffer_rsrc((void*)(p.A + (long long)m0 * p.lda * 2), 0, (int)abytes, 0x00020000);
        } else a_rs = __builtin_amdgcn_make_buffer_rsrc((void*)p.A, 0, 0, 0x00020000);
        a_so = 0;
    };
    auto setup_w = [&](int idx) __attribute__((always_inline)) {
        if (idx < count) {
            int m0, n0, mt;
            decode(idx, m0, n0, mt);
            if (p.ldw == 0) {
                w_rs = __builtin_amdgcn_make_buffer_rsrc((void*)(p.W + (long long)(n0 >> 8) * p.nt * V_TILE), 0, p.nt * V_TILE, 0x00020000);
            } else {
                const long long wbytes = (255LL * p.ldw + p.K) * 2;
                w_rs = __builtin_amdgcn_make_buffer_rsrc((void*)(p.W + (long long)n0 * p.ldw * 2), 0, (int)wbytes, 0x00020000);
            }
        } else w_rs = __builtin_amdgcn_make_buffer_rsrc((void*)p.W, 0, 0, 0x00020000);
        w_so = 0;
    };
    auto setup_src = [&](int idx) { setup_a(idx); setup_w(idx); };
    auto dma = [&](int stg, int q) __attribute__((always_inline)) {
        char* dst = lds + stg * V_STAGE + (q >= 4 ? V_TILE : 0) + (wave * 4 + (q & 3)) * 1024;
        if (q < 4) __builtin_amdgcn_raw_ptr_buffer_load_lds(a_rs, (void __attribute__((address_space(3)))*)dst, 16, avo[q & 3], a_so, 0, 0);
        else __builtin_amdgcn_raw_ptr_buffer_load_lds(w_rs, (void __attribute__((address_space(3)))*)dst, 16, wvo[q & 3], w_so, 0, 0);
    };
    auto advance = [&]() __attribute__((always_inline)) { a_so += 64; w_so += w_kstride; };
    auto next_src = [&](int idx) __attribute__((always_inline)) { setup_src(idx); };
    auto dma_a = [&](int slot, int i) __attribute__((always_inline)) {
        char* dst = lds + slot * X_ASLOT + (wave * 8 + i) * 1024;
        __builtin_amdgcn_raw_ptr_buffer_load_lds(a_rs, (void __attribute__((address_space(3)))*)dst, 16, avo[i & 1], a_so + i * a_rows8, 0, 0);
    };
    auto dma_w = [&](int stg, int j) __attribute__((always_inline)) {
        char* dst = lds + X_WBASE + stg * V_TILE + (wave * 4 + j) * 1024;
        __builtin_amdgcn_raw_ptr_buffer_load_lds(w_rs, (void __attribute__((address_space(3)))*)dst, 16, wvo[j], w_so, 0, 0);
    };

    const char* bias_lds = lds + V_RING;
    if constexpr (q_has_bias<EPI>() && !AW) {
        const int ncols = p.tiles_n * 256;
        for (int i = tid * 8; i < ncols; i += 256 * 8) {
            bf16x8 v = bf16x8{0, 0, 0, 0, 0, 0, 0, 0};
            if (p.bias && i < p.N) v = *reinterpret_cast<const bf16x8*>(p.bias + i);
            *reinterpret_cast<bf16x8*>(lds + V_RING + i * 2) = v;
        }
        asm volatile("s_waitcnt lgkmcnt(0)" ::: "memory");
    }

    const unsigned lds_base = (unsigned)(uintptr_t)((__attribute__((address_space(3))) char*)lds);
    unsigned a_rd, w_rd;
    unsigned a_rd1 = 0;
    {
        const int fi = lane & 15, fg = lane >> 4;
        const int fpos = fg ^ v_swz(fi >> 2);
        if constexpr (AW) {
            const int xpos = fg ^ ((fi >> 1) & 7);
            a_rd = lds_base + (wm * 128 + fi) * 128 + xpos * 16;
            a_rd1 = lds_base + (wm * 128 + fi) * 128 + (xpos ^ 4) * 16;
            w_rd = lds_base + X_WBASE + (wn * 128 + fi) * 64 + fpos * 16;
        } else {
            a_rd = lds_base + (wm * 128 + fi) * 64 + fpos * 16;
            w_rd = lds_base + V_TILE + (wn * 128 + fi) * 64 + fpos * 16;
        }
    }
    constexpr int A_FRAG = AW ? 2048 : 1024;
    int sp = 0;

    int stg = 0;
    bf16x8 xa[8], wa[8], xb[8], wb[8];
    f32x4 acc[8][8];
#ifdef NTW_PROBE
    v_f32x16 acc32[16];
    if constexpr (ABL & 8) {
#pragma unroll
        for (int i = 0; i < 16; ++i) acc32[i] = v_f32x16{0.f, 0.f, 0.f, 0.f, 0.f, 0.f, 0.f, 0.f, 0.f, 0.f, 0.f, 0.f, 0.f, 0.f, 0.f, 0.f};
    }
#endif

#ifdef NTW_PROBE
#define V_MFMA32(G, I_, XC, WC) do { if constexpr (!(ABL & 4) && (ABL & 8)) v_mfma32(acc32[(2 * (G) + (I_)) & 15], XC[(G) >> 1], WC[((G) & 1) * 4 + (I_)]); } while (0)
#else
#define V_MFMA32(G, I_, XC, WC) do { } while (0)
#endif
#define V_GROUP(G, Z, XC, WC, XN, WN) do { \
        constexpr int fm_ = (G) >> 1, h_ = ((G) & 1) * 4; \
        if constexpr (!(ABL & 4) && !(ABL & 8)) v_mfma<Z>(acc[h_ + 0][fm_], XC[fm_], WC[h_ + 0]); \
        V_MFMA32(G, 0, XC, WC); \
        if constexpr (!(ABL & 2)) { if constexpr ((G) < 8) XN[(G)] = v_rd<(G) * A_FRAG>(rdA); else WN[(G) - 8] = v_rd<((G) - 8) * 1024>(rdW); } \
        if constexpr (!(ABL & 4) && !(ABL & 8)) v_mfma<Z>(acc[h_ + 1][fm_], XC[fm_], WC[h_ + 1]); \
        if constexpr (!(ABL & 4) && !(ABL & 8)) v_mfma<Z>(acc[h_ + 2][fm_], XC[fm_], WC[h_ + 2]); \
        if constexpr (!(ABL & 1) && ((G) & 1)) { V_PIN(); if constexpr (AW) { if constexpr ((G) < 8) dma_a(dslot_, di0_ + ((G) >> 1)); else dma_w(stg, ((G) >> 1) - 4); } else dma(stg, (G) >> 1); V_PIN(); } \
        V_MFMA32(G, 1, XC, WC); \
        if constexpr (!(ABL & 4) && !(ABL & 8)) v_mfma<Z>(acc[h_ + 3][fm_], XC[fm_], WC[h_ + 3]); \
    } while (0)
#define V_STEP(Z, XC, WC, XN, WN, WAIT, H) do { \
        const unsigned soff_ = ((stg + 1) & 3) * (AW ? V_TILE : V_STAGE); \
        const int sp1_ = sp == 2 ? 0 : sp + 1; \
        const int dslot_ = (H) ? sp : (sp == 0 ? 2 : sp - 1); \
        constexpr int di0_ = (H) ? 0 : 4; \
        const unsigned rdA = AW ? ((H) ? a_rd + sp1_ * X_ASLOT : a_rd1 + sp * X_ASLOT) : a_rd + soff_; \
        const unsigned rdW = w_rd + soff_; \
        __builtin_amdgcn_s_setprio(1); \
        V_GROUP(0, Z, XC, WC, XN, WN); V_GROUP(1, Z, XC, WC, XN, WN); V_GROUP(2, Z, XC, WC, XN, WN); V_GROUP(3, Z, XC, WC, XN, WN); \
        V_GROUP(4, Z, XC, WC, XN, WN); V_GROUP(5, Z, XC, WC, XN, WN); V_GROUP(6, Z, XC, WC, XN, WN); V_GROUP(7, Z, XC, WC, XN, WN); \
        V_GROUP(8, Z, XC, WC, XN, WN); V_GROUP(9, Z, XC, WC, XN, WN); V_GROUP(10, Z, XC, WC, XN, WN); V_GROUP(11, Z, XC, WC, XN, WN); \
        V_GROUP(12, Z, XC, WC, XN, WN); V_GROUP(13, Z, XC, WC, XN, WN); V_GROUP(14, Z, XC, WC, XN, WN); V_GROUP(15, Z, XC, WC, XN, WN); \
        __builtin_amdgcn_s_setprio(0); \
        asm volatile("s_waitcnt lgkmcnt(0)" ::: "memory");       \
        if constexpr (!(ABL & 1)) { WAIT; } \
        V_PIN(); \
        __builtin_amdgcn_s_barrier();            \
        V_PIN(); \
        if constexpr (!(ABL & 1)) { if constexpr (AW) { w_so += w_kstride; if constexpr (!(H)) a_so += 128; } else advance(); } \
        if constexpr (AW && (H)) sp = sp1_; \
        stg = (stg + 1) & 3; \
    } while (0)
#define V_WAIT16 asm volatile("s_waitcnt vmcnt(16)" ::: "memory")
    bf16x4 bq[2] = {bf16x4{0, 0, 0, 0}, bf16x4{0, 0, 0, 0}};
    auto epilogue = [&](int m0, int n0, int mt) __attribute__((always_inline)) {
        constexpr int NR = 16;
#ifdef NTW_PROBE
        if constexpr (ABL & 8) {
#pragma unroll
            for (int i = 0; i < 16; ++i) asm volatile("" :: "a"(acc32[i]));
            return;
        }
#endif
        if (p.dbg & 1) {
#pragma unroll
            for (int i = 0; i < 8; ++i)
#pragma unroll
                for (int j = 0; j < 8; ++j) asm volatile("" :: "a"(acc[i][j]));
            return;
        }
        int elane;
        asm volatile("v_mbcnt_lo_u32_b32 %0, -1, 0\n\tv_mbcnt_hi_u32_b32 %0, -1, %0" : "=v"(elane));
        int fi = elane & 15, fg = elane >> 4, ewm = wm, ewn = wn;
        asm volatile("" : "+v"(fi), "+v"(fg), "+s"(ewm), "+s"(ewn));
        const int mrow0 = m0 + ewm * 128 + 4 * fg;
        const int ncolw = n0 + ewn * 128;
        const long long obase4 = (long long)mrow0 * p.ldc + ncolw + 4 * fi;
        f32x4 b4[2] = {f32x4{0.f, 0.f, 0.f, 0.f}, f32x4{0.f, 0.f, 0.f, 0.f}};
        if constexpr (q_has_bias<EPI>()) {
            if constexpr (AW) asm volatile("" : "+v"(bq[0]), "+v"(bq[1]));
#pragma unroll
            for (int qq = 0; qq < 2; ++qq) {
                bf16x4 bb;
                if constexpr (AW) bb = bq[qq];
                else bb = *reinterpret_cast<const bf16x4*>(bias_lds + (ncolw + qq * 64 + 4 * fi) * 2);
                b4[qq] = f32x4{(float)bb[0], (float)bb[1], (float)bb[2], (float)bb[3]};
            }
        }
        if constexpr (F32OUT) {
            float* Cf = reinterpret_cast<float*>(p.C);
            const float* Rf = reinterpret_cast<const float*>(p.resid);
            constexpr int D = 4;
            f32x4 r[D][4];
            auto fetch = [&](int rr_, f32x4 (&dst)[4]) __attribute__((always_inline)) {
                const int f = rr_ >> 1, qq = rr_ & 1;
                long long orow = obase4 + (long long)(f * 16) * p.ldc + qq * 64;
                asm volatile("" : "+v"(orow));
                const float* rp = Rf + orow;
#pragma unroll
                for (int j = 0; j < 4; ++j) q_gload_f32x4(dst[j], rp + (long long)j * p.ldc);
            };
#pragma unroll
            for (int i = 0; i < D; ++i) fetch(i, r[i]);
            auto row = [&](auto rc) __attribute__((always_inline)) {
                constexpr int R_ = decltype(rc)::value;
                constexpr int f = R_ >> 1, qq = R_ & 1;
                V_PIN();
                asm volatile("" : "+a"(acc[4 * qq + 0][f]), "+a"(acc[4 * qq + 1][f]), "+a"(acc[4 * qq + 2][f]), "+a"(acc[4 * qq + 3][f]));
                f32x4 (&rr)[4] = r[R_ % D];
                q_wait_regs4<q_epi_younger(R_, NR, D, 4)>(rr[0], rr[1], rr[2], rr[3]);
                long long ocp = obase4 + (long long)(f * 16) * p.ldc + qq * 64;
                asm volatile("" : "+v"(ocp));
                float* cp = Cf + ocp;
#pragma unroll
                for (int j = 0; j < 4; ++j) {
                    f32x4 v = f32x4{acc[4 * qq + 0][f][j], acc[4 * qq + 1][f][j], acc[4 * qq + 2][f][j], acc[4 * qq + 3][f][j]} + b4[qq];
                    v += rr[j];
                    *reinterpret_cast<f32x4*>(cp + (long long)j * p.ldc) = v;
                }
                if constexpr (R_ + D < NR) fetch(R_ + D, rr);
            };
            row(std::integral_constant<int, 0>{}); row(std::integral_constant<int, 1>{}); row(std::integral_constant<int, 2>{}); row(std::integral_constant<int, 3>{});
            row(std::integral_constant<int, 4>{}); row(std::integral_constant<int, 5>{}); row(std::integral_constant<int, 6>{}); row(std::integral_constant<int, 7>{});
            row(std::integral_constant<int, 8>{}); row(std::integral_constant<int, 9>{}); row(std::integral_constant<int, 10>{}); row(std::integral_constant<int, 11>{});
            row(std::integral_constant<int, 12>{}); row(std::integral_constant<int, 13>{}); row(std::integral_constant<int, 14>{}); row(std::integral_constant<int, 15>{});
        } else if constexpr (EPI == VITK_EPI_RESID16) {
            __bf16* Cb = reinterpret_cast<__bf16*>(p.C);
            const __bf16* Rb = reinterpret_cast<const __bf16*>(p.resid);
            constexpr int D = 6;
            bf16x4 r[D][4];
            auto fetch = [&](int rr_, bf16x4 (&dst)[4]) __attribute__((always_inline)) {
                const int f = rr_ >> 1, qq = rr_ & 1;
                long long orow = obase4 + (long long)(f * 16) * p.ldc + qq * 64;
                asm volatile("" : "+v"(orow));
                const __bf16* rp = Rb + orow;
#pragma unroll
                for (int j = 0; j < 4; ++j) v_gload_bf16x4(dst[j], rp + (long long)j * p.ldc);
            };
#pragma unroll
            for (int i = 0; i < D; ++i) fetch(i, r[i]);
            auto row = [&](auto rc) __attribute__((always_inline)) {
                constexpr int R_ = decltype(rc)::value;
                constexpr int f = R_ >> 1, qq = R_ & 1;
                V_PIN();
                asm volatile("" : "+a"(acc[4 * qq + 0][f]), "+a"(acc[4 * qq + 1][f]), "+a"(acc[4 * qq + 2][f]), "+a"(acc[4 * qq + 3][f]));
                bf16x4 (&rr)[4] = r[R_ % D];
                q_wait_regs4<q_epi_younger(R_, NR, D, 4)>(rr[0], rr[1], rr[2], rr[3]);
                long long ocp = obase4 + (long long)(f * 16) * p.ldc + qq * 64;
                asm volatile("" : "+v"(ocp));
                __bf16* cp = Cb + ocp;
#pragma unroll
                for (int j = 0; j < 4; ++j) {
                    f32x4 v = f32x4{acc[4 * qq + 0][f][j], acc[4 * qq + 1][f][j], acc[4 * qq + 2][f][j], acc[4 * qq + 3][f][j]} + b4[qq];
                    const bf16x4 q4 = rr[j];
                    v += f32x4{(float)q4[0], (float)q4[1], (float)q4[2], (float)q4[3]};
                    store4<__bf16>(cp + (long long)j * p.ldc, v);
                }
                if constexpr (R_ + D < NR) fetch(R_ + D, rr);
            };
            row(std::integral_constant<int, 0>{}); row(std::integral_constant<int, 1>{}); row(std::integral_constant<int, 2>{}); row(std::integral_constant<int, 3>{});
            row(std::integral_constant<int, 4>{}); row(std::integral_constant<int, 5>{}); row(std::integral_constant<int, 6>{}); row(std::integral_constant<int, 7>{});
            row(std::integral_constant<int, 8>{}); row(std::integral_constant<int, 9>{}); row(std::integral_constant<int, 10>{}); row(std::integral_constant<int, 11>{});
            row(std::integral_constant<int, 12>{}); row(std::integral_constant<int, 13>{}); row(std::integral_constant<int, 14>{}); row(std::integral_constant<int, 15>{});
        } else {
            const int odd = fi & 1;
            __bf16* Cb = reinterpret_cast<__bf16*>(p.C);
            const long long obase = (long long)(mrow0 + odd) * p.ldc + ncolw + 8 * (fi >> 1);
            constexpr bool AUX_IN = q_aux_in<EPI>();
            constexpr bool AUX8 = (EPI == VITK_EPI_MUL_AUX8);
            constexpr int DP = AUX8 ? 4 : 6;
            using HPre = std::conditional_t<AUX8, q_u32x2, bf16x8>;
            HPre hpre[DP][2];
            auto fetch_pre = [&](int rr_, HPre (&dst)[2]) __attribute__((always_inline)) {
                const int f = rr_ >> 1, qq = rr_ & 1;
                long long oa = obase + (long long)(f * 16) * p.ldc + qq * 64;
                asm volatile("" : "+v"(oa));
#pragma unroll
                for (int pr = 0; pr < 2; ++pr) {
                    if constexpr (AUX8) q_gload_u32x2(dst[pr], reinterpret_cast<const unsigned char*>(p.aux) + oa + (long long)(2 * pr) * p.ldc);
                    else q_gload_bf16x8(dst[pr], p.aux + oa + (long long)(2 * pr) * p.ldc);
                }
            };
            if constexpr (AUX_IN) {
#pragma unroll
                for (int i = 0; i < DP; ++i) fetch_pre(i, hpre[i]);
            }
            float cs[2][8];
#pragma unroll
            for (int e = 0; e < 8; ++e) { cs[0][e] = 0.f; cs[1][e] = 0.f; }
            auto frow = [&](auto rc) __attribute__((always_inline)) {
                constexpr int R_ = decltype(rc)::value;
                constexpr int f = R_ >> 1, qq = R_ & 1;
                V_PIN();
                asm volatile("" : "+a"(acc[4 * qq + 0][f]), "+a"(acc[4 * qq + 1][f]), "+a"(acc[4 * qq + 2][f]), "+a"(acc[4 * qq + 3][f]));
                if constexpr (AUX_IN) q_wait_regs2<q_epi_younger(R_, NR, DP, 2)>(hpre[R_ % DP][0], hpre[R_ % DP][1]);
                long long o0 = obase + (long long)(f * 16) * p.ldc + qq * 64;
                asm volatile("" : "+v"(o0));
#pragma unroll
                for (int pr = 0; pr < 2; ++pr) {
                    const int j0 = 2 * pr;
                    const f32x4 bq = b4[qq];
                    const unsigned a0 = q_pack2b<q_has_bias<EPI>()>(acc[4 * qq + 0][f][j0], acc[4 * qq + 1][f][j0], bq[0], bq[1]);
                    const unsigned a1 = q_pack2b<q_has_bias<EPI>()>(acc[4 * qq + 2][f][j0], acc[4 * qq + 3][f][j0], bq[2], bq[3]);
                    const unsigned c0 = q_pack2b<q_has_bias<EPI>()>(acc[4 * qq + 0][f][j0 + 1], acc[4 * qq + 1][f][j0 + 1], bq[0], bq[1]);
                    const unsigned c1 = q_pack2b<q_has_bias<EPI>()>(acc[4 * qq + 2][f][j0 + 1], acc[4 * qq + 3][f][j0 + 1], bq[2], bq[3]);
                    const unsigned r0 = q_dpp_xor1(odd ? a0 : c0), r1 = q_dpp_xor1(odd ? a1 : c1);
                    const unsigned k0 = odd ? c0 : a0, k1 = odd ? c1 : a1;
                    const q_u32x4 w4 = odd ? q_u32x4{r0, r1, k0, k1} : q_u32x4{k0, k1, r0, r1};
                    const bf16x8 v = __builtin_bit_cast(bf16x8, w4);
                    const long long o = o0 + (long long)j0 * p.ldc;
                    if constexpr (EPI == VITK_EPI_NONE || EPI == VITK_EPI_BIAS) {
                        *reinterpret_cast<bf16x8*>(Cb + o) = v;
                    } else if constexpr (EPI == VITK_EPI_BIAS_GELU) {
                        *reinterpret_cast<bf16x8*>(p.aux + o) = v;
                        *reinterpret_cast<bf16x8*>(Cb + o) = q_narrow8(q_gelu8(q_widen8(v)));
                    } else if constexpr (EPI == VITK_EPI_BIAS_GELU_DG || EPI == VITK_EPI_BIAS_GELU_DG8) {
                        q_f32x8 gl, dgl;
#ifdef NTW_PROBE
                        if (p.dbg & 32) { gl = q_widen8(v); dgl = gl; } else
#endif
                        q_gelu_both8(q_widen8(v), gl, dgl);
#ifdef NTW_PROBE
                        if (p.dbg & 64) { const bf16x8 t0 = q_narrow8(gl); const q_u32x2 t1 = q_dg_encode8(dgl); asm volatile("" :: "v"(t0), "v"(t1)); continue; }
#endif
                        if constexpr (EPI == VITK_EPI_BIAS_GELU_DG8) *reinterpret_cast<q_u32x2*>(reinterpret_cast<unsigned char*>(p.aux) + o) = q_dg_encode8(dgl);
                        else *reinterpret_cast<bf16x8*>(p.aux + o) = q_narrow8(dgl);
                        *reinterpret_cast<bf16x8*>(Cb + o) = q_narrow8(gl);
                    } else if constexpr (AUX_IN) {
                        q_f32x8 fac;
                        if constexpr (AUX8) fac = q_dg_decode8(hpre[R_ % DP][pr]);
                        else if constexpr (EPI == VITK_EPI_MUL_AUX) fac = q_widen8(hpre[R_ % DP][pr]);
                        else fac = q_gelu_grad8(q_widen8(hpre[R_ % DP][pr]));
                        const q_f32x8 g = q_widen8(v) * fac;
                        const bf16x8 g8 = q_narrow8(g);
#ifdef NTW_PROBE
                        if (p.dbg & 64) asm volatile("" :: "v"(g8)); else
#endif
                        *reinterpret_cast<bf16x8*>(Cb + o) = g8;
                        q_cs_add8(cs[qq], g8);
                    }
                }
                if constexpr (AUX_IN) {
                    if constexpr (R_ + DP < NR) fetch_pre(R_ + DP, hpre[R_ % DP]);
                }
            };
            frow(std::integral_constant<int, 0>{}); frow(std::integral_constant<int, 1>{}); frow(std::integral_constant<int, 2>{}); frow(std::integral_constant<int, 3>{});
            frow(std::integral_constant<int, 4>{}); frow(std::integral_constant<int, 5>{}); frow(std::integral_constant<int, 6>{}); frow(std::integral_constant<int, 7>{});
            frow(std::integral_constant<int, 8>{}); frow(std::integral_constant<int, 9>{}); frow(std::integral_constant<int, 10>{}); frow(std::integral_constant<int, 11>{});
            frow(std::integral_constant<int, 12>{}); frow(std::integral_constant<int, 13>{}); frow(std::integral_constant<int, 14>{}); frow(std::integral_constant<int, 15>{});
            if constexpr (AUX_IN) {
                if (p.csum) {
#pragma unroll
                    for (int qq = 0; qq < 2; ++qq) {
#pragma unroll
                        for (int e = 0; e < 8; ++e) {
                            float v = cs[qq][e];
                            v += __builtin_bit_cast(float, q_dpp_xor1(__builtin_bit_cast(unsigned, v)));
                            unsigned u = __builtin_bit_cast(unsigned, v);
                            auto a = __builtin_amdgcn_permlane16_swap(u, u, false, false);
                            v = __builtin_bit_cast(float, (unsigned)a[0]) + __builtin_bit_cast(float, (unsigned)a[1]);
                            u = __builtin_bit_cast(unsigned, v);
                            auto b = __builtin_amdgcn_permlane32_swap(u, u, false, false);
                            cs[qq][e] = __builtin_bit_cast(float, (unsigned)b[0]) + __builtin_bit_cast(float, (unsigned)b[1]);
                        }
                        if (fg == 0 && !odd) {
                            float* cp = p.csum + (long long)(2 * mt + ewm) * p.N + ncolw + qq * 64 + 8 * (fi >> 1);
                            *reinterpret_cast<f32x4*>(cp) = f32x4{cs[qq][0], cs[qq][1], cs[qq][2], cs[qq][3]};
                            *reinterpret_cast<f32x4*>(cp + 4) = f32x4{cs[qq][4], cs[qq][5], cs[qq][6], cs[qq][7]};
                        }
                    }
                }
            }
        }
    };

    setup_src(l0);
    if constexpr (!(ABL & 1)) {
        if constexpr (AW) {
#pragma unroll
            for (int pr = 0; pr < 2; ++pr) {
#pragma unroll
                for (int i = 0; i < 8; ++i) dma_a(pr, i);
                a_so += 128;
#pragma unroll
                for (int k = 0; k < 2; ++k) {
#pragma unroll
                    for (int j = 0; j < 4; ++j) dma_w(2 * pr + k, j);
                    w_so += w_kstride;
                }
            }
#pragma unroll
            for (int i = 0; i < 4; ++i) dma_a(2, i);
            asm volatile("s_waitcnt vmcnt(20)" ::: "memory");
        } else {
#pragma unroll
            for (int s = 0; s < 4; ++s) {
#pragma unroll
                for (int q = 0; q < 8; ++q) dma(s, q);
                advance();
            }
            asm volatile("s_waitcnt vmcnt(16)" ::: "memory");
        }
    }
    V_PIN();
    __builtin_amdgcn_s_barrier();
    V_PIN();
    {
        const unsigned rdA = a_rd, rdW = w_rd;
        xa[0] = v_rd<0 * A_FRAG>(rdA); xa[1] = v_rd<1 * A_FRAG>(rdA); xa[2] = v_rd<2 * A_FRAG>(rdA); xa[3] = v_rd<3 * A_FRAG>(rdA);
        xa[4] = v_rd<4 * A_FRAG>(rdA); xa[5] = v_rd<5 * A_FRAG>(rdA); xa[6] = v_rd<6 * A_FRAG>(rdA); xa[7] = v_rd<7 * A_FRAG>(rdA);
        wa[0] = v_rd<0 * 1024>(rdW); wa[1] = v_rd<1 * 1024>(rdW); wa[2] = v_rd<2 * 1024>(rdW); wa[3] = v_rd<3 * 1024>(rdW);
        wa[4] = v_rd<4 * 1024>(rdW); wa[5] = v_rd<5 * 1024>(rdW); wa[6] = v_rd<6 * 1024>(rdW); wa[7] = v_rd<7 * 1024>(rdW);
        asm volatile("s_waitcnt lgkmcnt(0)" ::: "memory");
    }
    V_PIN();
    __builtin_amdgcn_s_barrier();
    V_PIN();
    if constexpr (ABL & 2) {
#pragma unroll
        for (int f = 0; f < 8; ++f) { xb[f] = xa[f]; wb[f] = wa[f]; }
    }

    constexpr int ST_ROW = (F32OUT || EPI == VITK_EPI_RESID16 || q_two_outputs<EPI>()) ? 4 : 2;
    constexpr int VM_RELAX = 16 + 16 * ST_ROW > 63 ? 63 : 16 + 16 * ST_ROW;
    constexpr bool RELAX_OK = (EPI == VITK_EPI_NONE || (EPI == VITK_EPI_BIAS && !AW));
    bool relax = false;
#define V_WAITR do { \
        if (relax) asm volatile("s_waitcnt vmcnt(%0)" :: "n"(VM_RELAX) : "memory"); \
        else asm volatile("s_waitcnt vmcnt(16)" ::: "memory"); \
    } while (0)

    for (int idx = l0; idx < count; idx += L) {
        int m0, n0, mt;
        decode(idx, m0, n0, mt);
        if constexpr (AW && q_has_bias<EPI>()) {
            if (p.bias) {
                const __bf16* bp = p.bias + n0 + wn * 128 + 4 * (lane & 15);
                v_gload_bf16x4(bq[0], bp);
                v_gload_bf16x4(bq[1], bp + 64);
            }
        }
        V_STEP(true, xa, wa, xb, wb, V_WAITR, 0);
        V_STEP(false, xb, wb, xa, wa, V_WAITR, 1);
        if constexpr (AW) {
            for (int kt = 2; kt + 6 < p.nt; kt += 2) {
                V_STEP(false, xa, wa, xb, wb, V_WAIT16, 0);
                V_STEP(false, xb, wb, xa, wa, V_WAIT16, 1);
            }
            V_STEP(false, xa, wa, xb, wb, V_WAIT16, 0);
            setup_a(idx + L);
            V_STEP(false, xb, wb, xa, wa, V_WAIT16, 1);
            setup_w(idx + L);
            V_STEP(false, xa, wa, xb, wb, V_WAIT16, 0);
            V_STEP(false, xb, wb, xa, wa, V_WAIT16, 1);
            V_STEP(false, xa, wa, xb, wb, V_WAIT16, 0);
            V_STEP(false, xb, wb, xa, wa, V_WAIT16, 1);
        } else {
            for (int kt = 2; kt + 4 < p.nt; kt += 2) {
                V_STEP(false, xa, wa, xb, wb, V_WAIT16, 0);
                V_STEP(false, xb, wb, xa, wa, V_WAIT16, 1);
            }
            next_src(idx + L);
            V_STEP(false, xa, wa, xb, wb, V_WAIT16, 0);
            V_STEP(false, xb, wb, xa, wa, V_WAIT16, 1);
            V_STEP(false, xa, wa, xb, wb, V_WAIT16, 0);
            V_STEP(false, xb, wb, xa, wa, V_WAIT16, 1);
        }
        asm volatile("s_nop 15\n\ts_nop 15" ::: "memory");
        V_PIN();
        epilogue(m0, n0, mt);
        relax = (RELAX_OK || (p.dbg & 16)) && !(p.dbg & 3);
    }
    asm volatile("s_waitcnt vmcnt(0)" ::: "memory");
#undef V_WAITR
#undef V_WAIT16
#undef V_STEP
#undef V_GROUP
#undef V_MFMA32
}

template <typename Kern>
int v_set_max_lds(Kern kernel, int bytes) {
    return (int)hipFuncSetAttribute(reinterpret_cast<const void*>(kernel), hipFuncAttributeMaxDynamicSharedMemorySize, bytes);
}

}

bool gemm_ntw_serves(int64_t M, int64_t N, int64_t K) {
    return !((K % 64) || K < 256 || (N % 256) || M < 256 || N > 16128 || (K / 32) * (long long)V_TILE >= (1LL << 31));
}

int gemm_ntw_split(int64_t M, int64_t N, int64_t K, int grid) {
    const long long tiles_n = N / 256;
    const long long tm_cap = (M % 256 == 0) ? M / 256 : (M - 1024) / 256;
    if (tm_cap <= 0) return 0;
    double second_launch = 14.0 / (0.72 * (double)(K / 32) + 6.0);
    if (const char* e = vitk_exp("VITK_NTW_SPLIT")) second_launch = e[0] == 'r' ? 0.15 : (e[0] == 'n' ? 100.0 : second_launch);
    auto legal = [&](long long tm) { const long long rest = M - 256 * tm; return tm > 0 && tm <= tm_cap && (rest == 0 || rest >= 1024); };
    auto cost = [&](long long tm) -> double {
        const long long rest = M - 256 * tm;
        double c = (double)((tm * tiles_n + grid - 1) / grid);
        if (rest > 0) c += second_launch + 0.6 * (double)((((rest + 127) / 128) * tiles_n + grid - 1) / grid);
        return c;
    };
    long long best_tm = 0;
    double best = 1e30;
    auto consider = [&](long long tm) { if (legal(tm)) { const double c = cost(tm); if (c < best) { best = c; best_tm = tm; } } };
    consider(tm_cap);
    if (M % 256 == 0 && tm_cap > 4) consider(tm_cap - 4);
    const long long k = (tm_cap * tiles_n) / grid;
    if (k >= 1) { long long tm = (k * grid) / tiles_n; consider(tm); while (tm > 0 && !legal(tm)) --tm; consider(tm); }
    if (vitk_exp("VITK_NTW_TM")) { const long long v = atoll(vitk_exp("VITK_NTW_TM")); if (v == 0 || legal(v)) best_tm = v; }
    return (int)best_tm;
}

int gemm_ntw_launch(int tiles_m, int grid, const void* A, int64_t lda, const void* W, int64_t ldw, void* C, int64_t ldc,
                    int64_t N, int64_t K, int epilogue, const void* bias, const void* resid, void* aux, float* csum, int abl, int dbg, void* stream) {
    NtwArgs a;
    a.A = (const char*)A; a.lda = lda; a.W = (const char*)W; a.ldw = ldw; a.C = C; a.ldc = ldc;
    a.M = 256 * tiles_m; a.N = (int)N; a.K = (int)K;
    a.bias = (const __bf16*)bias; a.resid = resid; a.aux = (__bf16*)aux; a.csum = csum;
    a.tiles_n = (int)(N / 256); a.tiles_m = tiles_m; a.n_tiles = a.tiles_m * a.tiles_n; a.nt = (int)(K / 32);
    a.group_n = a.tiles_n;
    if (a.tiles_n > 8) a.group_n = K <= 768 ? 4 : (a.tiles_n + (a.tiles_n + 5) / 6 - 1) / ((a.tiles_n + 5) / 6);
    if (vitk_exp("VITK_GROUP_N")) { const int g = atoi(vitk_exp("VITK_GROUP_N")); a.group_n = g > 0 && g < a.tiles_n ? g : a.tiles_n; }
    a.dbg = dbg;
    if (const char* e = vitk_exp("VITK_NTW_RELAX")) a.dbg |= e[0] == 'a' ? 16 : (e[0] == 'n' ? 2 : 0);
    const int lds_bytes = V_RING + a.tiles_n * 512 + 16;
    hipStream_t st = (hipStream_t)stream;
    if (tiles_m <= 0 || grid < 8) VITK_FAIL(VITK_E_ARG, "gemm_nt_bf16 (w128): nothing to do");
    const char* aw_e = vitk_switch("VITK_NTW_A128");
    const bool a128 = !(aw_e && aw_e[0] == '0');
#define NTW_LAUNCH1(E, AB) do { \
        if (a128) { \
            static const int rc1__ = v_set_max_lds(gemm_ntw_kernel<E, AB, 1>, X_LDS); \
            if (rc1__ != 0) VITK_FAIL(rc1__, "gemm_nt_bf16 (w128): cannot enable %d B of LDS", X_LDS); \
            hipLaunchKernelGGL((gemm_ntw_kernel<E, AB, 1>), dim3((unsigned)grid), dim3(256), X_LDS, st, a); \
        } else { \
            static const int rc__ = v_set_max_lds(gemm_ntw_kernel<E, AB, 0>, V_LDS_MAX); \
            if (rc__ != 0) VITK_FAIL(rc__, "gemm_nt_bf16 (w128): cannot enable %d B of LDS", V_LDS_MAX); \
            hipLaunchKernelGGL((gemm_ntw_kernel<E, AB, 0>), dim3((unsigned)grid), dim3(256), lds_bytes, st, a); \
        } \
    } while (0)
#ifdef NTW_PROBE
#define NTW_LAUNCH_ALL(E) do { \
        switch (abl) { \
            case 0: NTW_LAUNCH1(E, 0); break; case 1: NTW_LAUNCH1(E, 1); break; case 2: NTW_LAUNCH1(E, 2); break; case 3: NTW_LAUNCH1(E, 3); break; \
            case 4: NTW_LAUNCH1(E, 4); break; case 5: NTW_LAUNCH1(E, 5); break; case 6: NTW_LAUNCH1(E, 6); break; case 7: NTW_LAUNCH1(E, 7); break; \
            case 8: NTW_LAUNCH1(E, 8); break; case 10: NTW_LAUNCH1(E, 10); break; case 11: NTW_LAUNCH1(E, 11); break; \
            default: VITK_FAIL(VITK_E_ARG, "gemm_nt_bf16 (w128): bad ablation %d", abl); \
        } } while (0)
#define NTW_LAUNCH(E) do { if (abl == 0) NTW_LAUNCH1(E, 0); else if (abl == 7) NTW_LAUNCH1(E, 7); else VITK_FAIL(VITK_E_ARG, "gemm_nt_bf16 (w128): ablation %d exists for EPI_NONE only", abl); } while (0)
#else
#define NTW_LAUNCH(E) do { if (abl) VITK_FAIL(VITK_E_ARG, "gemm_nt_bf16 (w128): ablations exist in tools/nt_probe.hip only"); NTW_LAUNCH1(E, 0); } while (0)
#define NTW_LAUNCH_ALL(E) NTW_LAUNCH(E)
#endif
    switch (epilogue) {
        case VITK_EPI_NONE: NTW_LAUNCH_ALL(VITK_EPI_NONE); break;
#ifndef NTW_PROBE_LEAN
        case VITK_EPI_BIAS: NTW_LAUNCH(VITK_EPI_BIAS); break;
        case VITK_EPI_BIAS_GELU: NTW_LAUNCH(VITK_EPI_BIAS_GELU); break;
        case VITK_EPI_RESID: NTW_LAUNCH(VITK_EPI_RESID); break;
        case VITK_EPI_GELU_BWD: NTW_LAUNCH(VITK_EPI_GELU_BWD); break;
        case VITK_EPI_BIAS_GELU_DG: NTW_LAUNCH(VITK_EPI_BIAS_GELU_DG); break;
        case VITK_EPI_MUL_AUX: NTW_LAUNCH(VITK_EPI_MUL_AUX); break;
        case VITK_EPI_BIAS_GELU_DG8: NTW_LAUNCH(VITK_EPI_BIAS_GELU_DG8); break;
        case VITK_EPI_MUL_AUX8: NTW_LAUNCH(VITK_EPI_MUL_AUX8); break;
        case VITK_EPI_RESID16: NTW_LAUNCH(VITK_EPI_RESID16); break;
#endif
        default: VITK_FAIL(VITK_E_ARG, "gemm_nt_bf16 (w128): bad epilogue %d", epilogue);
    }
#undef NTW_LAUNCH_ALL
#undef NTW_LAUNCH
#undef NTW_LAUNCH1
    VITK_CHECK_LAUNCH("gemm_nt_bf16 (w128)");
    return 0;
}
```

Measured before the change: 8827.

## Add 128-row half tiles to persistent w128 NT GEMM with makespan planner

Extends the persistent 256x256 NT GEMM kernel so it can also process 128-row half tiles in the same launch, replacing the separate fallback launch for leftover rows. A makespan model picks how many full versus half tiles to assign per XCD to balance work across CUs. Non-colsum, non-dropout epilogues now take this single-launch path. This removes the second-launch cost and tail imbalance, at the price of more kernel code size and a cost model that may be mis-tuned.

Result: faster. 9004 (median of 6 runs) (+2.0%).

```diff
diff --git a/include/vitk.h b/include/vitk.h
--- a/include/vitk.h
+++ b/include/vitk.h
@@ -81,6 +81,7 @@
 int vitk_gemm_nt_bf16_mul_aux8_colsum(const void* A, int64_t lda, const void* W, int64_t ldw, void* C, int64_t ldc,
                                       int64_t M, int64_t N, int64_t K, const void* aux8, float* colsum_partials, void* stream);
 int vitk_gemm_nt_plan(int64_t M, int64_t N, int64_t K, int64_t ldc, int32_t* out5);
+int vitk_gemm_nt_w128_plan(int64_t M, int64_t N, int64_t K, int32_t grid, int32_t* out4);
 int64_t vitk_pack_w_nt_bytes(int64_t rows, int64_t reduction);
 int vitk_pack_w_nt(const void* W, int64_t ldw, int64_t N, int64_t K, void* out, void* out_t, void* stream);
 int vitk_pack_w_nt_many(const void* const* W, const int64_t* ldw, const int64_t* N, const int64_t* K, void* const* out,
diff --git a/vit_pytorch_amd/_lib.py b/vit_pytorch_amd/_lib.py
--- a/vit_pytorch_amd/_lib.py
+++ b/vit_pytorch_amd/_lib.py
@@ -68,6 +68,7 @@
     "vitk_gemm_tn_fp8": (_i, [_vp, _i64, _vp, _i64, _vp, _i, _i64, _i, _i64, _i64, _i64, _vp, _i64, _vp, _vp, _i, _vp]),
     "vitk_gemm_nt_colsum_rows": (_i64, [_i64, _i64, _i64, _i64]),
     "vitk_gemm_nt_plan": (_i, [_i64, _i64, _i64, _i64, _vp]),
+    "vitk_gemm_nt_w128_plan": (_i, [_i64, _i64, _i64, _i, _vp]),
     "vitk_comm_unique_id": (_i, [_vp]),
     "vitk_comm_init": (_i, [_vp, _i, _i, _vp]),
     "vitk_comm_allreduce": (_i, [_vp, _vp, _i64, _i, _i, _vp]),
diff --git a/vit_pytorch_amd/csrc/gemm_bf16.hip b/vit_pytorch_amd/csrc/gemm_bf16.hip
--- a/vit_pytorch_amd/csrc/gemm_bf16.hip
+++ b/vit_pytorch_amd/csrc/gemm_bf16.hip
@@ -725,6 +725,22 @@
     return 0;
 }
 
+extern "C" int vitk_gemm_nt_w128_plan(int64_t M, int64_t N, int64_t K, int32_t grid, int32_t* out4) {
+    if (!out4) VITK_FAIL(VITK_E_ARG, "gemm_nt_w128_plan: null output");
+    for (int i = 0; i < 4; ++i) out4[i] = 0;
+    if (grid < 8 || (grid & 7)) VITK_FAIL(VITK_E_ARG, "gemm_nt_w128_plan: grid must be a positive multiple of 8 (got %d)", grid);
+    int tm = 0, th = 0;
+    if (M <= 0 || N <= 0 || K <= 0 || !gemm_ntw_plan(M, N, K, grid, &tm, &th)) return 0;
+    out4[0] = tm; out4[1] = th;
+    out4[2] = (int32_t)(1000.0 * gemm_ntw_makespan(N, K, grid, tm, th) + 0.5);
+    const int ts = gemm_ntw_split(M, N, K, grid);
+    const int64_t rest = M - 256LL * ts, tiles_n = N / 256;
+    double old = gemm_ntw_makespan(N, K, grid, ts, 0);
+    if (rest > 0) old += 14.0 / (0.72 * (double)(K / 32) + 6.0) + 0.6 * (double)((((rest + 127) / 128) * tiles_n + grid - 1) / grid);
+    out4[3] = (int32_t)(1000.0 * old + 0.5);
+    return 0;
+}
+
 extern "C" int vitk_gemm_nt_bf16_gelu_bwd_colsum(const void* A, int64_t lda, const void* W, int64_t ldw, void* C, int64_t ldc,
                                                  int64_t M, int64_t N, int64_t K, void* aux, float* colsum_partials, void* stream) {
     if (!colsum_partials) VITK_FAIL(VITK_E_ARG, "gemm_nt_bf16_gelu_bwd_colsum: null partials");
@@ -750,12 +766,15 @@
 }
 
 constexpr unsigned NTW_EPIS = 0xffu;
-static int ntw_tiles_m(const NtpPlan& q, int64_t M, int64_t N, int64_t K, int epilogue, int grid = 0) {
+static bool ntw_enabled(const NtpPlan& q, int64_t M, int64_t N, int64_t K, int epilogue) {
     if (epilogue == VITK_EPI_BIAS_GELU_DG8) epilogue = VITK_EPI_BIAS_GELU_DG;
     if (epilogue == VITK_EPI_MUL_AUX8) epilogue = VITK_EPI_MUL_AUX;
     const char* e = vitk_switch("VITK_NT_W128");
     const unsigned mask = e ? (unsigned)strtoul(e, nullptr, 0) : NTW_EPIS;
-    if (!q.ok || !((mask >> epilogue) & 1u) || !gemm_ntw_serves(M, N, K)) return 0;
+    return q.ok && ((mask >> epilogue) & 1u) && gemm_ntw_serves(M, N, K);
+}
+static int ntw_tiles_m(const NtpPlan& q, int64_t M, int64_t N, int64_t K, int epilogue, int grid = 0) {
+    if (!ntw_enabled(q, M, N, K, epilogue)) return 0;
     return gemm_ntw_split(M, N, K, grid > 0 ? grid : q.grid);
 }
 static int64_t nt_persist_colsum_rows(const NtpPlan& q, int64_t M, int64_t N, int64_t K, int64_t ldc) {
@@ -770,6 +789,12 @@
     const int reserve = vitk_get_cu_reserve();
     int grid_w = q.grid - (reserve + 7) / 8 * 8;
     if (grid_w < q.grid / 4) grid_w = q.grid / 4 / 8 * 8;
+    const bool colsum_epi = epilogue == VITK_EPI_GELU_BWD || epilogue == VITK_EPI_MUL_AUX || epilogue == VITK_EPI_MUL_AUX8;
+    int tm1 = 0, th1 = 0;
+    if (!colsum_epi && !drop_t && ntw_enabled(q, M, N, K, epilogue) && gemm_ntw_plan(M, N, K, grid_w, &tm1, &th1)) {
+        if (256LL * (lda > ldw ? lda : ldw) * 2 + K * 2 >= (1LL << 31)) VITK_FAIL(VITK_E_SHAPE, "gemm_nt_bf16: row stride too large (lda %lld, ldw %lld)", (long long)lda, (long long)ldw);
+        return gemm_ntw_launch(tm1, grid_w, A, lda, W, ldw, C, ldc, N, K, epilogue, bias, resid, aux, csum, 0, 0, stream, th1);
+    }
     const int tmw = ntw_tiles_m(q, M, N, K, epilogue == VITK_EPI_GELU_BWD ? VITK_EPI_MUL_AUX : epilogue, csum ? 0 : grid_w);
     const int64_t asz = (epilogue == VITK_EPI_BIAS_GELU_DG8 || epilogue == VITK_EPI_MUL_AUX8) ? 1 : 2;
     if (tmw == 0 || (drop_t && !(epilogue == VITK_EPI_GELU_BWD && csum)))
diff --git a/vit_pytorch_amd/csrc/gemm_nt_plan.h b/vit_pytorch_amd/csrc/gemm_nt_plan.h
--- a/vit_pytorch_amd/csrc/gemm_nt_plan.h
+++ b/vit_pytorch_amd/csrc/gemm_nt_plan.h
@@ -21,5 +21,9 @@
 
 bool gemm_ntw_serves(int64_t M, int64_t N, int64_t K);
 int gemm_ntw_split(int64_t M, int64_t N, int64_t K, int grid);
+bool gemm_ntw_plan(int64_t M, int64_t N, int64_t K, int grid, int* tiles_m, int* tiles_mh);
+double gemm_ntw_half_cost(int64_t K);
+double gemm_ntw_makespan(int64_t N, int64_t K, int grid, int64_t tiles_m, int64_t tiles_mh);
 int gemm_ntw_launch(int tiles_m, int grid, const void* A, int64_t lda, const void* W, int64_t ldw, void* C, int64_t ldc,
-                    int64_t N, int64_t K, int epilogue, const void* bias, const void* resid, void* aux, float* csum, int abl, int dbg, void* stream);
+                    int64_t N, int64_t K, int epilogue, const void* bias, const void* resid, void* aux, float* csum, int abl, int dbg, void* stream,
+                    int tiles_mh = 0);
diff --git a/vit_pytorch_amd/csrc/gemm_nt_w128.hip b/vit_pytorch_amd/csrc/gemm_nt_w128.hip
--- a/vit_pytorch_amd/csrc/gemm_nt_w128.hip
+++ b/vit_pytorch_amd/csrc/gemm_nt_w128.hip
@@ -2,6 +2,7 @@
 #include "gemm_nt_plan.h"
 #include "gemm_nt_epi.h"
 #include <stdlib.h>
+#include <algorithm>
 #include <type_traits>
 
 #ifdef VITK_HALF_IS_F16
@@ -41,6 +42,7 @@
     int M, N, K;
     const __bf16* bias; const void* resid; __bf16* aux; float* csum;
     int tiles_n, group_n, tiles_m, n_tiles, nt;
+    int tiles_mh, n_half;
     int dbg;
 };
 
@@ -76,14 +78,23 @@
     const int wave = __builtin_amdgcn_readfirstlane(tid >> 6);
     const int wm = wave >> 1, wn = wave & 1;
 
+    constexpr bool HALF_OK = !q_aux_in<EPI>() && ABL == 0;
     const int xcd = blockIdx.x & 7, l0 = blockIdx.x >> 3, L = gridDim.x >> 3;
     const int ms = (int)(((long long)xcd * p.n_tiles) >> 3), count = (int)(((long long)(xcd + 1) * p.n_tiles) >> 3) - ms;
-    if (l0 >= count) return;
+    const int hs = HALF_OK ? (int)(((long long)xcd * p.n_half) >> 3) : 0;
+    const int total = HALF_OK ? count + (int)(((long long)(xcd + 1) * p.n_half) >> 3) - hs : count;
+    if (l0 >= total) return;
     if ((p.dbg >> 8) && (l0 & 1)) { for (int i = (p.dbg >> 8) & 0xff; i > 0; --i) __builtin_amdgcn_s_sleep(127); }
-    auto decode = [&](int idx, int& m0, int& n0, int& mt) {
+    auto decode = [&](int idx, int& m0, int& n0, int& mt) -> bool {
         int tn;
-        v_grouped_tile(ms + idx, p.tiles_m, p.tiles_n, p.group_n, mt, tn);
-        m0 = mt * 256; n0 = tn * 256;
+        if (!HALF_OK || idx < count) {
+            v_grouped_tile(ms + idx, p.tiles_m, p.tiles_n, p.group_n, mt, tn);
+            m0 = mt * 256; n0 = tn * 256;
+            return false;
+        }
+        v_grouped_tile(hs + idx - count, p.tiles_mh, p.tiles_n, p.group_n, mt, tn);
+        m0 = 256 * p.tiles_m + 128 * mt; n0 = tn * 256;
+        return true;
     };
 
     const int srow = lane >> 2, spos = lane & 3;
@@ -100,16 +111,19 @@
     __amdgpu_buffer_rsrc_t a_rs, w_rs;
     int a_so = 0, w_so = 0;
     auto setup_a = [&](int idx) __attribute__((always_inline)) {
-        if (idx < count) {
+        if (idx < total) {
             int m0, n0, mt;
-            decode(idx, m0, n0, mt);
-            const long long abytes = (255LL * p.lda + p.K) * 2;
+            long long abytes = (255LL * p.lda + p.K) * 2;
+            if (decode(idx, m0, n0, mt)) {
+                m0 -= 64 * (wave >> 1);
+                abytes = (wave & 1) ? 0 : ((64LL * wave + 63) * p.lda + p.K) * 2;
+            }
             a_rs = __builtin_amdgcn_make_buffer_rsrc((void*)(p.A + (long long)m0 * p.lda * 2), 0, (int)abytes, 0x00020000);
         } else a_rs = __builtin_amdgcn_make_buffer_rsrc((void*)p.A, 0, 0, 0x00020000);
         a_so = 0;
     };
     auto setup_w = [&](int idx) __attribute__((always_inline)) {
-        if (idx < count) {
+        if (idx < total) {
             int m0, n0, mt;
             decode(idx, m0, n0, mt);
             if (p.ldw == 0) {
@@ -184,18 +198,18 @@
 #else
 #define V_MFMA32(G, I_, XC, WC) do { } while (0)
 #endif
-#define V_GROUP(G, Z, XC, WC, XN, WN) do { \
-        constexpr int fm_ = (G) >> 1, h_ = ((G) & 1) * 4; \
+#define V_GROUP(G, Z, XC, WC, XN, WN, HF, HR) do { \
+        constexpr int fm_ = (HF) ? (G) >> 2 : (G) >> 1, h_ = (HF) ? ((G) & 3) * 2 : ((G) & 1) * 4; \
         if constexpr (!(ABL & 4) && !(ABL & 8)) v_mfma<Z>(acc[h_ + 0][fm_], XC[fm_], WC[h_ + 0]); \
         V_MFMA32(G, 0, XC, WC); \
-        if constexpr (!(ABL & 2)) { if constexpr ((G) < 8) XN[(G)] = v_rd<(G) * A_FRAG>(rdA); else WN[(G) - 8] = v_rd<((G) - 8) * 1024>(rdW); } \
+        if constexpr (!(ABL & 2)) { if constexpr ((G) < 8) { if constexpr (!((HR) && (G) >= 4)) XN[(G)] = v_rd<(G) * A_FRAG>(rdA); } else WN[(G) - 8] = v_rd<((G) - 8) * 1024>(rdW); } \
         if constexpr (!(ABL & 4) && !(ABL & 8)) v_mfma<Z>(acc[h_ + 1][fm_], XC[fm_], WC[h_ + 1]); \
-        if constexpr (!(ABL & 4) && !(ABL & 8)) v_mfma<Z>(acc[h_ + 2][fm_], XC[fm_], WC[h_ + 2]); \
+        if constexpr (!(ABL & 4) && !(ABL & 8) && !(HF)) v_mfma<Z>(acc[(HF) ? 0 : h_ + 2][fm_], XC[fm_], WC[(HF) ? 0 : h_ + 2]); \
         if constexpr (!(ABL & 1) && ((G) & 1)) { V_PIN(); if constexpr (AW) { if constexpr ((G) < 8) dma_a(dslot_, di0_ + ((G) >> 1)); else dma_w(stg, ((G) >> 1) - 4); } else dma(stg, (G) >> 1); V_PIN(); } \
         V_MFMA32(G, 1, XC, WC); \
-        if constexpr (!(ABL & 4) && !(ABL & 8)) v_mfma<Z>(acc[h_ + 3][fm_], XC[fm_], WC[h_ + 3]); \
+        if constexpr (!(ABL & 4) && !(ABL & 8) && !(HF)) v_mfma<Z>(acc[(HF) ? 0 : h_ + 3][fm_], XC[fm_], WC[(HF) ? 0 : h_ + 3]); \
     } while (0)
-#define V_STEP(Z, XC, WC, XN, WN, WAIT, H) do { \
+#define V_STEP(Z, XC, WC, XN, WN, WAIT, H, HF, HR) do { \
         const unsigned soff_ = ((stg + 1) & 3) * (AW ? V_TILE : V_STAGE); \
         const int sp1_ = sp == 2 ? 0 : sp + 1; \
         const int dslot_ = (H) ? sp : (sp == 0 ? 2 : sp - 1); \
@@ -203,10 +217,10 @@
         const unsigned rdA = AW ? ((H) ? a_rd + sp1_ * X_ASLOT : a_rd1 + sp * X_ASLOT) : a_rd + soff_; \
         const unsigned rdW = w_rd + soff_; \
         __builtin_amdgcn_s_setprio(1); \
-        V_GROUP(0, Z, XC, WC, XN, WN); V_GROUP(1, Z, XC, WC, XN, WN); V_GROUP(2, Z, XC, WC, XN, WN); V_GROUP(3, Z, XC, WC, XN, WN); \
-        V_GROUP(4, Z, XC, WC, XN, WN); V_GROUP(5, Z, XC, WC, XN, WN); V_GROUP(6, Z, XC, WC, XN, WN); V_GROUP(7, Z, XC, WC, XN, WN); \
-        V_GROUP(8, Z, XC, WC, XN, WN); V_GROUP(9, Z, XC, WC, XN, WN); V_GROUP(10, Z, XC, WC, XN, WN); V_GROUP(11, Z, XC, WC, XN, WN); \
-        V_GROUP(12, Z, XC, WC, XN, WN); V_GROUP(13, Z, XC, WC, XN, WN); V_GROUP(14, Z, XC, WC, XN, WN); V_GROUP(15, Z, XC, WC, XN, WN); \
+        V_GROUP(0, Z, XC, WC, XN, WN, HF, HR); V_GROUP(1, Z, XC, WC, XN, WN, HF, HR); V_GROUP(2, Z, XC, WC, XN, WN, HF, HR); V_GROUP(3, Z, XC, WC, XN, WN, HF, HR); \
+        V_GROUP(4, Z, XC, WC, XN, WN, HF, HR); V_GROUP(5, Z, XC, WC, XN, WN, HF, HR); V_GROUP(6, Z, XC, WC, XN, WN, HF, HR); V_GROUP(7, Z, XC, WC, XN, WN, HF, HR); \
+        V_GROUP(8, Z, XC, WC, XN, WN, HF, HR); V_GROUP(9, Z, XC, WC, XN, WN, HF, HR); V_GROUP(10, Z, XC, WC, XN, WN, HF, HR); V_GROUP(11, Z, XC, WC, XN, WN, HF, HR); \
+        V_GROUP(12, Z, XC, WC, XN, WN, HF, HR); V_GROUP(13, Z, XC, WC, XN, WN, HF, HR); V_GROUP(14, Z, XC, WC, XN, WN, HF, HR); V_GROUP(15, Z, XC, WC, XN, WN, HF, HR); \
         __builtin_amdgcn_s_setprio(0); \
         asm volatile("s_waitcnt lgkmcnt(0)" ::: "memory");       \
         if constexpr (!(ABL & 1)) { WAIT; } \
@@ -219,8 +233,9 @@
     } while (0)
 #define V_WAIT16 asm volatile("s_waitcnt vmcnt(16)" ::: "memory")
     bf16x4 bq[2] = {bf16x4{0, 0, 0, 0}, bf16x4{0, 0, 0, 0}};
-    auto epilogue = [&](int m0, int n0, int mt) __attribute__((always_inline)) {
-        constexpr int NR = 16;
+    auto epilogue = [&](int m0, int n0, int mt, auto hc) __attribute__((always_inline)) {
+        constexpr bool HF = decltype(hc)::value;
+        constexpr int NR = HF ? 8 : 16;
 #ifdef NTW_PROBE
         if constexpr (ABL & 8) {
 #pragma unroll
@@ -239,7 +254,7 @@
         asm volatile("v_mbcnt_lo_u32_b32 %0, -1, 0\n\tv_mbcnt_hi_u32_b32 %0, -1, %0" : "=v"(elane));
         int fi = elane & 15, fg = elane >> 4, ewm = wm, ewn = wn;
         asm volatile("" : "+v"(fi), "+v"(fg), "+s"(ewm), "+s"(ewn));
-        const int mrow0 = m0 + ewm * 128 + 4 * fg;
+        const int mrow0 = m0 + ewm * (HF ? 64 : 128) + 4 * fg;
         const int ncolw = n0 + ewn * 128;
         const long long obase4 = (long long)mrow0 * p.ldc + ncolw + 4 * fi;
         f32x4 b4[2] = {f32x4{0.f, 0.f, 0.f, 0.f}, f32x4{0.f, 0.f, 0.f, 0.f}};
@@ -288,8 +303,10 @@
             };
             row(std::integral_constant<int, 0>{}); row(std::integral_constant<int, 1>{}); row(std::integral_constant<int, 2>{}); row(std::integral_constant<int, 3>{});
             row(std::integral_constant<int, 4>{}); row(std::integral_constant<int, 5>{}); row(std::integral_constant<int, 6>{}); row(std::integral_constant<int, 7>{});
-            row(std::integral_constant<int, 8>{}); row(std::integral_constant<int, 9>{}); row(std::integral_constant<int, 10>{}); row(std::integral_constant<int, 11>{});
-            row(std::integral_constant<int, 12>{}); row(std::integral_constant<int, 13>{}); row(std::integral_constant<int, 14>{}); row(std::integral_constant<int, 15>{});
+            if constexpr (!HF) {
+                row(std::integral_constant<int, 8>{}); row(std::integral_constant<int, 9>{}); row(std::integral_constant<int, 10>{}); row(std::integral_constant<int, 11>{});
+                row(std::integral_constant<int, 12>{}); row(std::integral_constant<int, 13>{}); row(std::integral_constant<int, 14>{}); row(std::integral_constant<int, 15>{});
+            }
         } else if constexpr (EPI == VITK_EPI_RESID16) {
             __bf16* Cb = reinterpret_cast<__bf16*>(p.C);
             const __bf16* Rb = reinterpret_cast<const __bf16*>(p.resid);
@@ -326,8 +343,10 @@
             };
             row(std::integral_constant<int, 0>{}); row(std::integral_constant<int, 1>{}); row(std::integral_constant<int, 2>{}); row(std::integral_constant<int, 3>{});
             row(std::integral_constant<int, 4>{}); row(std::integral_constant<int, 5>{}); row(std::integral_constant<int, 6>{}); row(std::integral_constant<int, 7>{});
-            row(std::integral_constant<int, 8>{}); row(std::integral_constant<int, 9>{}); row(std::integral_constant<int, 10>{}); row(std::integral_constant<int, 11>{});
-            row(std::integral_constant<int, 12>{}); row(std::integral_constant<int, 13>{}); row(std::integral_constant<int, 14>{}); row(std::integral_constant<int, 15>{});
+            if constexpr (!HF) {
+                row(std::integral_constant<int, 8>{}); row(std::integral_constant<int, 9>{}); row(std::integral_constant<int, 10>{}); row(std::integral_constant<int, 11>{});
+                row(std::integral_constant<int, 12>{}); row(std::integral_constant<int, 13>{}); row(std::integral_constant<int, 14>{}); row(std::integral_constant<int, 15>{});
+            }
         } else {
             const int odd = fi & 1;
             __bf16* Cb = reinterpret_cast<__bf16*>(p.C);
@@ -412,8 +431,10 @@
             };
             frow(std::integral_constant<int, 0>{}); frow(std::integral_constant<int, 1>{}); frow(std::integral_constant<int, 2>{}); frow(std::integral_constant<int, 3>{});
             frow(std::integral_constant<int, 4>{}); frow(std::integral_constant<int, 5>{}); frow(std::integral_constant<int, 6>{}); frow(std::integral_constant<int, 7>{});
-            frow(std::integral_constant<int, 8>{}); frow(std::integral_constant<int, 9>{}); frow(std::integral_constant<int, 10>{}); frow(std::integral_constant<int, 11>{});
-            frow(std::integral_constant<int, 12>{}); frow(std::integral_constant<int, 13>{}); frow(std::integral_constant<int, 14>{}); frow(std::integral_constant<int, 15>{});
+            if constexpr (!HF) {
+                frow(std::integral_constant<int, 8>{}); frow(std::integral_constant<int, 9>{}); frow(std::integral_constant<int, 10>{}); frow(std::integral_constant<int, 11>{});
+                frow(std::integral_constant<int, 12>{}); frow(std::integral_constant<int, 13>{}); frow(std::integral_constant<int, 14>{}); frow(std::integral_constant<int, 15>{});
+            }
             if constexpr (AUX_IN) {
                 if (p.csum) {
 #pragma unroll
@@ -496,7 +517,40 @@
         else asm volatile("s_waitcnt vmcnt(16)" ::: "memory"); \
     } while (0)
 
-    for (int idx = l0; idx < count; idx += L) {
+#define V_TILE_STEPS(HF) do { \
+         \
+        V_STEP(true, xa, wa, xb, wb, V_WAITR, 0, HF, HF); \
+        V_STEP(false, xb, wb, xa, wa, V_WAITR, 1, HF, HF); \
+        if constexpr (AW) { \
+            for (int kt = 2; kt + 6 < p.nt; kt += 2) { \
+                V_STEP(false, xa, wa, xb, wb, V_WAIT16, 0, HF, HF); \
+                V_STEP(false, xb, wb, xa, wa, V_WAIT16, 1, HF, HF); \
+            } \
+            V_STEP(false, xa, wa, xb, wb, V_WAIT16, 0, HF, HF);      \
+            setup_a(idx + L);                                        \
+            V_STEP(false, xb, wb, xa, wa, V_WAIT16, 1, HF, HF); \
+            setup_w(idx + L);                                        \
+            V_STEP(false, xa, wa, xb, wb, V_WAIT16, 0, HF, HF); \
+            V_STEP(false, xb, wb, xa, wa, V_WAIT16, 1, HF, HF); \
+            V_STEP(false, xa, wa, xb, wb, V_WAIT16, 0, HF, HF); \
+            V_STEP(false, xb, wb, xa, wa, V_WAIT16, 1, HF, false);   \
+        } else { \
+            for (int kt = 2; kt + 4 < p.nt; kt += 2) { \
+                V_STEP(false, xa, wa, xb, wb, V_WAIT16, 0, HF, HF); \
+                V_STEP(false, xb, wb, xa, wa, V_WAIT16, 1, HF, HF); \
+            } \
+            next_src(idx + L);        \
+            V_STEP(false, xa, wa, xb, wb, V_WAIT16, 0, HF, HF); \
+            V_STEP(false, xb, wb, xa, wa, V_WAIT16, 1, HF, HF); \
+            V_STEP(false, xa, wa, xb, wb, V_WAIT16, 0, HF, HF); \
+            V_STEP(false, xb, wb, xa, wa, V_WAIT16, 1, HF, false);   \
+        } \
+         \
+        asm volatile("s_nop 15\n\ts_nop 15" ::: "memory"); \
+        V_PIN(); \
+    } while (0)
+    int idx = l0;
+    for (; idx < count; idx += L) {
         int m0, n0, mt;
         decode(idx, m0, n0, mt);
         if constexpr (AW && q_has_bias<EPI>()) {
@@ -506,38 +560,28 @@
                 v_gload_bf16x4(bq[1], bp + 64);
             }
         }
-        V_STEP(true, xa, wa, xb, wb, V_WAITR, 0);
-        V_STEP(false, xb, wb, xa, wa, V_WAITR, 1);
-        if constexpr (AW) {
-            for (int kt = 2; kt + 6 < p.nt; kt += 2) {
-                V_STEP(false, xa, wa, xb, wb, V_WAIT16, 0);
-                V_STEP(false, xb, wb, xa, wa, V_WAIT16, 1);
-            }
-            V_STEP(false, xa, wa, xb, wb, V_WAIT16, 0);
-            setup_a(idx + L);
-            V_STEP(false, xb, wb, xa, wa, V_WAIT16, 1);
-            setup_w(idx + L);
-            V_STEP(false, xa, wa, xb, wb, V_WAIT16, 0);
-            V_STEP(false, xb, wb, xa, wa, V_WAIT16, 1);
-            V_STEP(false, xa, wa, xb, wb, V_WAIT16, 0);
-            V_STEP(false, xb, wb, xa, wa, V_WAIT16, 1);
-        } else {
-            for (int kt = 2; kt + 4 < p.nt; kt += 2) {
-                V_STEP(false, xa, wa, xb, wb, V_WAIT16, 0);
-                V_STEP(false, xb, wb, xa, wa, V_WAIT16, 1);
-            }
-            next_src(idx + L);
-            V_STEP(false, xa, wa, xb, wb, V_WAIT16, 0);
-            V_STEP(false, xb, wb, xa, wa, V_WAIT16, 1);
-            V_STEP(false, xa, wa, xb, wb, V_WAIT16, 0);
-            V_STEP(false, xb, wb, xa, wa, V_WAIT16, 1);
-        }
-        asm volatile("s_nop 15\n\ts_nop 15" ::: "memory");
-        V_PIN();
-        epilogue(m0, n0, mt);
+        V_TILE_STEPS(false);
+        epilogue(m0, n0, mt, std::false_type{});
         relax = (RELAX_OK || (p.dbg & 16)) && !(p.dbg & 3);
     }
+    if constexpr (HALF_OK) {
+        for (; idx < total; idx += L) {
+            int m0, n0, mt;
+            decode(idx, m0, n0, mt);
+            if constexpr (AW && q_has_bias<EPI>()) {
+                if (p.bias) {
+                    const __bf16* bp = p.bias + n0 + wn * 128 + 4 * (lane & 15);
+                    v_gload_bf16x4(bq[0], bp);
+                    v_gload_bf16x4(bq[1], bp + 64);
+                }
+            }
+            V_TILE_STEPS(true);
+            epilogue(m0, n0, mt, std::true_type{});
+            relax = false;
+        }
+    }
     asm volatile("s_waitcnt vmcnt(0)" ::: "memory");
+#undef V_TILE_STEPS
 #undef V_WAITR
 #undef V_WAIT16
 #undef V_STEP
@@ -580,13 +624,47 @@
     return (int)best_tm;
 }
 
+double gemm_ntw_half_cost(int64_t K) {
+    const double nt = (double)(K / 32);
+    return (0.41 * nt + 4.2) / (0.72 * nt + 6.0);
+}
+double gemm_ntw_makespan(int64_t N, int64_t K, int grid, int64_t tiles_m, int64_t tiles_mh) {
+    const long long tiles_n = N / 256, nf = tiles_m * tiles_n, nh = tiles_mh * tiles_n, L = grid / 8;
+    const double h = gemm_ntw_half_cost(K);
+    double worst = 0.0;
+    for (long long x = 0; x < 8; ++x) {
+        const long long c = ((x + 1) * nf >> 3) - (x * nf >> 3), hc = ((x + 1) * nh >> 3) - (x * nh >> 3);
+        const long long q = c / L, r = c % L, hq = hc / L, hr = hc % L;
+        double w = (double)q + h * (double)(hq + (hr > 0 ? 1 : 0));
+        if (r > 0) w = std::max(w, (double)(q + 1) + h * (double)(hq + (hr > L - r ? 1 : 0)));
+        worst = std::max(worst, w);
+    }
+    return worst;
+}
+bool gemm_ntw_plan(int64_t M, int64_t N, int64_t K, int grid, int* tiles_m, int* tiles_mh) {
+    *tiles_m = 0; *tiles_mh = 0;
+    if (M % 128 || !gemm_ntw_serves(M, N, K) || grid < 8) return false;
+    const long long tiles_n = N / 256, units = M / 128, tm_all = units / 2;
+    const long long lo = std::max(0LL, tm_all - (grid + tiles_n - 1) / tiles_n - 1);
+    long long best_tm = tm_all;
+    double best = gemm_ntw_makespan(N, K, grid, tm_all, units - 2 * tm_all);
+    for (long long tm = tm_all - 1; tm >= lo; --tm) {
+        const double c = gemm_ntw_makespan(N, K, grid, tm, units - 2 * tm);
+        if (c < best - 1e-9) { best = c; best_tm = tm; }
+    }
+    *tiles_m = (int)best_tm; *tiles_mh = (int)(units - 2 * best_tm);
+    return true;
+}
+
 int gemm_ntw_launch(int tiles_m, int grid, const void* A, int64_t lda, const void* W, int64_t ldw, void* C, int64_t ldc,
-                    int64_t N, int64_t K, int epilogue, const void* bias, const void* resid, void* aux, float* csum, int abl, int dbg, void* stream) {
+                    int64_t N, int64_t K, int epilogue, const void* bias, const void* resid, void* aux, float* csum, int abl, int dbg, void* stream,
+                    int tiles_mh) {
     NtwArgs a;
     a.A = (const char*)A; a.lda = lda; a.W = (const char*)W; a.ldw = ldw; a.C = C; a.ldc = ldc;
-    a.M = 256 * tiles_m; a.N = (int)N; a.K = (int)K;
+    a.M = 256 * tiles_m + 128 * tiles_mh; a.N = (int)N; a.K = (int)K;
     a.bias = (const __bf16*)bias; a.resid = resid; a.aux = (__bf16*)aux; a.csum = csum;
     a.tiles_n = (int)(N / 256); a.tiles_m = tiles_m; a.n_tiles = a.tiles_m * a.tiles_n; a.nt = (int)(K / 32);
+    a.tiles_mh = tiles_mh; a.n_half = tiles_mh * a.tiles_n;
     a.group_n = a.tiles_n;
     if (a.tiles_n > 8) a.group_n = K <= 768 ? 4 : (a.tiles_n + (a.tiles_n + 5) / 6 - 1) / ((a.tiles_n + 5) / 6);
     if (vitk_exp("VITK_GROUP_N")) { const int g = atoi(vitk_exp("VITK_GROUP_N")); a.group_n = g > 0 && g < a.tiles_n ? g : a.tiles_n; }
@@ -594,7 +672,9 @@
     if (const char* e = vitk_exp("VITK_NTW_RELAX")) a.dbg |= e[0] == 'a' ? 16 : (e[0] == 'n' ? 2 : 0);
     const int lds_bytes = V_RING + a.tiles_n * 512 + 16;
     hipStream_t st = (hipStream_t)stream;
-    if (tiles_m <= 0 || grid < 8) VITK_FAIL(VITK_E_ARG, "gemm_nt_bf16 (w128): nothing to do");
+    if (tiles_m < 0 || tiles_mh < 0 || tiles_m + tiles_mh <= 0 || grid < 8) VITK_FAIL(VITK_E_ARG, "gemm_nt_bf16 (w128): nothing to do");
+    if (tiles_mh > 0 && (abl || epilogue == VITK_EPI_GELU_BWD || epilogue == VITK_EPI_MUL_AUX || epilogue == VITK_EPI_MUL_AUX8))
+        VITK_FAIL(VITK_E_ARG, "gemm_nt_bf16 (w128): 128-row tiles exist without column sums and ablations only");
     const char* aw_e = vitk_switch("VITK_NTW_A128");
     const bool a128 = !(aw_e && aw_e[0] == '0');
 #define NTW_LAUNCH1(E, AB) do { \
```
